# Lakonik/SSDNeRF

Measured on NVIDIA H100. Metric: rays/sec (128^2 render) & DDIM triplanes/sec, higher is better.
Workload: dtype fp16 tensor-core UNet (fp32 accumulate), fp32 renderer

## Files before the change

### include/ssdnerf_b200.h

```cpp
#ifndef SSDNERF_B200_H_
#define SSDNERF_B200_H_

#include <stdint.h>
#include <stddef.h>

#ifdef __cplusplus
extern "C" {
#endif

#define SSDNERF_API __attribute__((visibility("default")))

#define SSDNERF_OK 0
#define SSDNERF_ERR_CUDA (-1)
#define SSDNERF_ERR_ARG (-2)
#define SSDNERF_ERR_ARCH (-3)

SSDNERF_API const char* ssdnerf_last_error(void);
SSDNERF_API int ssdnerf_version(void);
SSDNERF_API int ssdnerf_compiled_arch(void);
SSDNERF_API unsigned long long ssdnerf_launch_count(void);

SSDNERF_API int ssdnerf_near_far_from_aabb(const float* rays_o, const float* rays_d, const float* aabb, uint32_t N, float min_near,
                               float* nears, float* fars, void* stream);
SSDNERF_API int ssdnerf_sph_from_ray(const float* rays_o, const float* rays_d, float radius, uint32_t N, float* coords, void* stream);
SSDNERF_API int ssdnerf_morton3D(const int* coords, uint32_t N, int* indices, void* stream);
SSDNERF_API int ssdnerf_morton3D_invert(const int* indices, uint32_t N, int* coords, void* stream);
SSDNERF_API int ssdnerf_packbits(const void* grid, int grid_is_half, uint32_t N, float thresh, uint8_t* bitfield, void* stream);
SSDNERF_API int ssdnerf_march_rays_train(const float* rays_o, const float* rays_d, const uint8_t* grid, float bound, float dt_gamma,
                             uint32_t max_steps, uint32_t N, uint32_t C, uint32_t H, uint32_t M, const float* nears,
                             const float* fars, float* xyzs, float* dirs, float* deltas, int* rays, int* counter,
                             const float* noises, void* stream);
SSDNERF_API int ssdnerf_composite_rays_train_forward(const float* sigmas, const float* rgbs, const float* deltas, const int* rays,
                                         uint32_t M, uint32_t N, float T_thresh, float* weights_sum, float* depth,
                                         float* image, void* stream);
SSDNERF_API int ssdnerf_composite_rays_train_backward(const float* grad_weights_sum, const float* grad_image, const float* sigmas,
                                          const float* rgbs, const float* deltas, const int* rays, const float* weights_sum,
                                          const float* image, uint32_t M, uint32_t N, float T_thresh, float* grad_sigmas,
                                          float* grad_rgbs, void* stream);
SSDNERF_API int ssdnerf_march_rays(uint32_t n_alive, uint32_t n_step, const int* rays_alive, const float* rays_t, const float* rays_o,
                       const float* rays_d, float bound, float dt_gamma, uint32_t max_steps, uint32_t C, uint32_t H,
                       const uint8_t* grid, const float* nears, const float* fars, float* xyzs, float* dirs, float* deltas,
                       const float* noises, void* stream);
SSDNERF_API int ssdnerf_composite_rays(uint32_t n_alive, uint32_t n_step, float T_thresh, int* rays_alive, float* rays_t,
                           const float* sigmas, const float* rgbs, const float* deltas, float* weights_sum, float* depth,
                           float* image, void* stream);
SSDNERF_API int ssdnerf_sh_encode_forward(const float* inputs, float* outputs, uint32_t B, uint32_t D, uint32_t C, int calc_grad_inputs,
                              float* dy_dx, void* stream);
SSDNERF_API int ssdnerf_sh_encode_backward(const float* grad, const float* inputs, uint32_t B, uint32_t D, uint32_t C, const float* dy_dx,
                               float* grad_inputs, void* stream);


#define SSDNERF_DEC_P 0
#define SSDNERF_DEC_S 1

SSDNERF_API size_t ssdnerf_decoder_blob_floats(int variant);

SSDNERF_API size_t ssdnerf_planes_bytes(int variant, uint32_t B, uint32_t Hp, uint32_t Wp);
SSDNERF_API int ssdnerf_pack_planes(int variant, const float* code, uint32_t B, uint32_t C, uint32_t Hp, uint32_t Wp, void* planes,
                        void* stream);

SSDNERF_API int ssdnerf_point_decode(int variant, const void* planes, uint32_t plane_h, uint32_t plane_w, const float* decoder_blob,
                                     const float* xyzs, const float* dirs, const long long* scene_offsets, uint32_t num_scenes,
                                     unsigned long long num_points, float* sigmas, float* rgbs, void* stream);

typedef struct ssdnerf_render_args {
    int variant;
    uint32_t num_scenes;
    uint32_t rays_per_scene;
    const float* rays_o;
    const float* rays_d;
    const float* poses;
    const float* intrinsics;
    uint32_t num_views, img_h, img_w;
    const void* planes;
    uint32_t plane_h, plane_w;
    const uint8_t* bitfield;
    uint32_t grid_size;
    const float* decoder_blob;
    const float* dt_gamma;
    float bound, min_near, T_thresh, bg_color;
    uint32_t max_steps;
    int emulate_schedule;
    float* weights_sum;
    float* depth;
    float* image;
    float* rgb_blend;
    int32_t* num_samples;
    int32_t* voxel_trace;
    uint32_t trace_cap;
    void* workspace;
    size_t workspace_bytes;
} ssdnerf_render_args;

SSDNERF_API size_t ssdnerf_render_workspace_bytes(uint32_t num_scenes, uint32_t rays_per_scene, uint32_t max_steps);
SSDNERF_API int ssdnerf_render_fwd(const ssdnerf_render_args* args, void* stream);

typedef struct ssdnerf_render_train_args {
    int variant;
    uint32_t num_scenes, rays_per_scene;
    const float* rays_o;
    const float* rays_d;
    const float* noises;
    const void* planes;
    uint32_t plane_h, plane_w;
    const uint8_t* bitfield;
    uint32_t grid_size;
    const float* decoder_blob;
    const float* dt_gamma;
    float bound, min_near, T_thresh;
    uint32_t max_steps;
    float* weights_sum;
    float* depth;
    float* image;
    int32_t* num_samples;
    const float* grad_ws;
    const float* grad_image;
    float* grad_planes;
    uint32_t* counter;
    float* grad_decoder_blob;
} ssdnerf_render_train_args;

SSDNERF_API int ssdnerf_cam_rays(const float* poses, const float* intrinsics, uint32_t B, uint32_t V, uint32_t h, uint32_t w,
                     float* rays_o, float* rays_d, void* stream);
SSDNERF_API int ssdnerf_render_train_fwd(const ssdnerf_render_train_args* args, void* stream);
SSDNERF_API int ssdnerf_render_train_bwd(const ssdnerf_render_train_args* args, void* stream);
SSDNERF_API int ssdnerf_unpack_plane_grads(const float* grad_planes, const float* code, float reg_coef, uint32_t B, uint32_t Hp, uint32_t Wp,
                               int accumulate, float* grad_code, void* stream);
SSDNERF_API int ssdnerf_mse_render_loss(const float* image, const float* weights_sum, const float* target, uint64_t rays, float bg_color,
                            float coef_loss, float coef_grad, float* out_rgb , float* grad_image, float* grad_ws,
                            float* loss , void* stream);

SSDNERF_API size_t ssdnerf_density_workspace_bytes(uint32_t num_scenes, uint32_t grid_size);
SSDNERF_API int ssdnerf_density_update(int variant, const void* planes, uint32_t plane_h, uint32_t plane_w, const float* decoder_blob,
                           uint32_t num_scenes, uint32_t grid_size, float bound,
                           const float* jitter,
                           float decay, void* density_grid, int grid_is_half, void* workspace, void* stream);
SSDNERF_API int ssdnerf_density_pack(const void* density_grid, int grid_is_half, uint32_t num_scenes, uint32_t grid_size,
                         float density_thresh, uint8_t* bitfield, float* thresh_out ,
                         void* workspace, void* stream);

typedef struct ssdnerf_gemm_args {
    const void* a1; uint64_t a1_strides[3]; uint32_t k1;
    const void* a2; uint64_t a2_strides[3]; uint32_t k2;
    uint32_t d1, d2, d3, b1, b2, b3;
    uint32_t taps;
    const void* b; uint64_t b_strides[3]; uint32_t n, n_rows_b, bx2, bx3; uint32_t b_batched;
    uint32_t bn;
    float alpha;
    const float* bias_n;
    const void* residual;
    void* out; uint32_t out_f32; long long so1, so2, so3;
    float* qstats; uint32_t stats_hw;
    uint32_t algo;
    const int8_t* tap_offsets;
    uint32_t a_stride;
    uint32_t relu;
} ssdnerf_gemm_args;
SSDNERF_API int ssdnerf_gemm_f16(const ssdnerf_gemm_args* args, void* stream);

SSDNERF_API int ssdnerf_nchw_to_nhwc_f16(const float* x, uint32_t B, uint32_t C, uint32_t H, uint32_t W, uint32_t Cpad, void* out, void* stream);
SSDNERF_API int ssdnerf_gn_stats(const void* x1, uint32_t C1, const void* x2, uint32_t C2, uint32_t B, uint32_t HW, uint32_t groups,
                                 float* stats, void* stream);
SSDNERF_API int ssdnerf_gn_apply_q(const void* x1, uint32_t C1, const void* x2, uint32_t C2, uint32_t B, uint32_t HW, uint32_t groups,
                                   const float* q1, const float* q2, const float* gamma, const float* beta, const float* scale_shift,
                                   long long ss_batch_stride, float eps, int do_silu, void* out, void* stream);
SSDNERF_API int ssdnerf_gn_apply(const void* x1, uint32_t C1, const void* x2, uint32_t C2, uint32_t B, uint32_t HW, uint32_t groups,
                                 const float* stats, const float* gamma, const float* beta, const float* scale_shift,
                                 long long ss_batch_stride, float eps, int do_silu, void* out, void* stream);
SSDNERF_API int ssdnerf_flash_attn(const void* qkv, uint32_t B, uint32_t T, uint32_t heads, uint32_t ch, float scale, void* out, void* stream);
SSDNERF_API int ssdnerf_softmax_rows(const float* S, uint32_t rows, uint32_t T, void* P, void* stream);
SSDNERF_API int ssdnerf_transpose_v(const void* qkv, uint32_t B, uint32_t T, uint32_t heads, uint32_t ch, void* vt, void* stream);
SSDNERF_API int ssdnerf_ddim_update(float* x_t, const float* v, uint32_t B, uint32_t C, uint32_t H, uint32_t W, uint32_t Cv,
                                    const float* coef, const int* step_ptr, int clip, float clip_lo, float clip_hi, float* x0_out,
                                    void* next_in, uint32_t Cpad, void* stream);
SSDNERF_API int ssdnerf_ddpm_update(float* x_t, const float* v, uint32_t B, uint32_t C, uint32_t H, uint32_t W, uint32_t Cv,
                                    const float* coef, const int* step_ptr, const unsigned long long* seed_ptr, int clip, float clip_lo,
                                    float clip_hi, void* next_in, uint32_t Cpad, void* stream);
SSDNERF_API int ssdnerf_step_counter(int* step_ptr, int value, int set, void* stream);
SSDNERF_API int ssdnerf_select_row(const float* table, uint32_t row_elems, const int* step_ptr, float* dst, uint32_t copies, void* stream);

typedef struct ssdnerf_gn_bwd_args {
    const void* x1; uint32_t C1;
    const void* x2; uint32_t C2;
    uint32_t B, HW, groups;
    const float* stats; const float* stats2; int quad_stats;
    const float* gamma; const float* beta;
    const float* scale_shift; long long ss_batch_stride;
    float eps; int do_silu;
    const void* dy;
    const void* add;
    float* group_sums;
    void* dx1; void* dx2;
    float* channel_sums;
} ssdnerf_gn_bwd_args;
SSDNERF_API int ssdnerf_gn_bwd(const ssdnerf_gn_bwd_args* args, void* stream);
SSDNERF_API int ssdnerf_softmax_bwd_rows(const void* P, const float* dP, uint32_t rows, uint32_t T, void* dS, void* stream);
SSDNERF_API int ssdnerf_transpose_f16(const void* src, void* dst, uint32_t rows, uint32_t cols, long long row_stride, long long stride1,
                                      uint32_t n1, long long stride2, uint32_t n2, void* stream);
SSDNERF_API int ssdnerf_col2im_s2(const void* dcol, uint32_t B, uint32_t H, uint32_t W, uint32_t C, const void* add, void* dx, void* stream);
SSDNERF_API int ssdnerf_sum2x2(const void* dup, uint32_t B, uint32_t H, uint32_t W, uint32_t C, void* dx, void* stream);
SSDNERF_API int ssdnerf_add_f16(void* dst, const void* src, unsigned long long n, void* stream);
SSDNERF_API int ssdnerf_grad_scale(const float* g, unsigned long long n, float target, float* scale, void* stream);
SSDNERF_API int ssdnerf_grad_nchw_to_nhwc_f16(const float* g, uint32_t B, uint32_t C, uint32_t H, uint32_t W, uint32_t Cpad, const float* scale,
                                              void* out, void* stream);
SSDNERF_API int ssdnerf_grad_nhwc_to_nchw_f32(const float* dx, uint32_t B, uint32_t C, uint32_t H, uint32_t W, uint32_t Cpad, float* scale,
                                              float* out, void* stream);


typedef struct ssdnerf_wgrad_args {
    const void* gy; uint32_t gy_stride, gy_c0;
    const void* x; uint32_t x_stride, x_c0;
    float* dw; uint32_t dw_stride, dw_c0;
    uint32_t batch, out_h, out_w, in_h, in_w;
    uint32_t cout, cin;
    uint32_t taps;
    uint32_t stride;
    int up;
    uint32_t ksplit;
} ssdnerf_wgrad_args;
SSDNERF_API int ssdnerf_conv_wgrad_f16(const ssdnerf_wgrad_args* args, void* stream);
SSDNERF_API int ssdnerf_dropout_f16(void* x, unsigned long long n, unsigned long long seed, float p_drop, void* stream);
SSDNERF_API int ssdnerf_colsum_f16(const void* src, uint64_t rows, uint32_t stride, uint32_t c0, uint32_t channels, float* out, void* stream);

SSDNERF_API int ssdnerf_ssim_f32(const float* pred, const float* target, uint32_t n, uint32_t h, uint32_t w, float* out, void* stream);
SSDNERF_API int ssdnerf_lpips_prep_f16(const float* pred, const float* target, uint32_t m, uint32_t h, uint32_t w, void* out, void* stream);
SSDNERF_API uint32_t ssdnerf_lpips_tap_partials(uint32_t m, uint32_t h, uint32_t w, uint32_t c, int pool);
SSDNERF_API int ssdnerf_lpips_tap_f16(const void* feat, uint32_t m, uint32_t h, uint32_t w, uint32_t c, const float* lin, float* partial,
                                     void* pooled, float* out, void* stream);

SSDNERF_API size_t ssdnerf_mc_workspace_bytes(uint32_t nx, uint32_t ny, uint32_t nz);
SSDNERF_API int ssdnerf_mc_count(const float* u, uint32_t nx, uint32_t ny, uint32_t nz, double threshold, void* workspace,
                                 unsigned long long* counts , void* stream);
SSDNERF_API int ssdnerf_mc_emit(const float* u, uint32_t nx, uint32_t ny, uint32_t nz, double threshold, const void* workspace,
                                double* vertices, long long* triangles, void* stream);
SSDNERF_API int ssdnerf_mc_case_table(uint8_t* tri_count_host, uint8_t* tri_host);

SSDNERF_API int ssdnerf_incep_prep_f16(const float* x, uint32_t n, uint32_t h, uint32_t w, void* out, uint8_t* u8, void* stream);
SSDNERF_API int ssdnerf_incep_conv_f16(const void* x, uint32_t n, uint32_t h, uint32_t w, uint32_t cin, uint32_t x_stride, const void* weight,
                                       const float* bias, uint32_t cout, uint32_t kh, uint32_t kw, uint32_t stride, uint32_t pad_h,
                                       uint32_t pad_w, int relu, void* y, uint32_t y_stride, void* stream);
#define SSDNERF_POOL_MAX_S2 0
#define SSDNERF_POOL_AVG_S1 1
#define SSDNERF_POOL_MAX_S1 2
SSDNERF_API int ssdnerf_incep_pool_f16(const void* x, uint32_t n, uint32_t h, uint32_t w, uint32_t c, uint32_t x_stride, int mode, void* y,
                                       uint32_t y_stride, void* stream);
SSDNERF_API int ssdnerf_incep_mean_f16(const void* x, uint32_t n, uint32_t hw, uint32_t c, float* out, void* stream);

#define SSDNERF_PNG_SEGMENT_BYTES 16384
SSDNERF_API size_t ssdnerf_png_workspace_bytes(uint32_t n, uint32_t h, uint32_t w);
SSDNERF_API size_t ssdnerf_png_output_bound(uint32_t n, uint32_t h, uint32_t w);
SSDNERF_API int ssdnerf_png_encode_views(const float* pred, const float* real, uint32_t n, uint32_t h, uint32_t w_view, void* workspace,
                                        size_t workspace_bytes, uint8_t* out, size_t out_bytes, unsigned long long* offsets,
                                        void* stream);
SSDNERF_API int ssdnerf_png_encode_maps(const float* maps, uint32_t n, uint32_t h, uint32_t w, float vmin, float vrange, void* workspace,
                                       size_t workspace_bytes, uint8_t* out, size_t out_bytes, unsigned long long* offsets,
                                       void* stream);
SSDNERF_API int ssdnerf_png_viridis(uint8_t* rgb_host);

#define SSDNERF_PNG_OK 0
#define SSDNERF_PNG_TRUNCATED 1
#define SSDNERF_PNG_BAD_ZLIB_HEADER 2
#define SSDNERF_PNG_BAD_BLOCK_TYPE 3
#define SSDNERF_PNG_BAD_STORED_LEN 4
#define SSDNERF_PNG_BAD_CODE_LENGTHS 5
#define SSDNERF_PNG_BAD_SYMBOL 6
#define SSDNERF_PNG_BAD_DISTANCE 7
#define SSDNERF_PNG_TOO_MUCH_DATA 8
#define SSDNERF_PNG_TOO_LITTLE_DATA 9
#define SSDNERF_PNG_BAD_FILTER 10
#define SSDNERF_PNG_BAD_ADLER 11
#define SSDNERF_PNG_BAD_DESC 12
typedef struct {
    uint64_t stream_offset;
    uint64_t palette_offset;
    uint64_t work_offset;
    uint64_t out_offset;
    uint32_t stream_bytes;
    uint32_t h, w;
    int32_t color_type;
} ssdnerf_png_desc;
SSDNERF_API size_t ssdnerf_png_decode_workspace_bytes(uint32_t h, uint32_t w, int color_type);
SSDNERF_API int ssdnerf_png_decode(const uint8_t* streams, size_t stream_bytes, const ssdnerf_png_desc* desc, uint32_t n, void* workspace,
                                   size_t workspace_bytes, float* out, size_t out_floats, int32_t* status, void* stream);
SSDNERF_API int ssdnerf_png_decode_host(const uint8_t* stream_host, size_t stream_bytes, uint32_t h, uint32_t w, int color_type,
                                        const uint8_t* palette_host, float* out_host, int32_t* status_host);

#ifdef __cplusplus
}
#endif
#endif
```

### ssdnerf_b200/_lib.py

```python
import ctypes
import os

import torch

_HERE = os.path.dirname(os.path.abspath(__file__))
_PATH = os.path.join(_HERE, 'libssdnerf_b200.so')
_lib = None

c_void_p = ctypes.c_void_p
c_u32 = ctypes.c_uint32
c_f32 = ctypes.c_float
c_double = ctypes.c_double
c_int = ctypes.c_int
c_size_t = ctypes.c_size_t
c_longlong = ctypes.c_longlong


class SSDNeRFNativeError(RuntimeError):
    pass


class RenderArgs(ctypes.Structure):
    _fields_ = [
        ('variant', c_int), ('num_scenes', c_u32), ('rays_per_scene', c_u32),
        ('rays_o', c_void_p), ('rays_d', c_void_p),
        ('poses', c_void_p), ('intrinsics', c_void_p),
        ('num_views', c_u32), ('img_h', c_u32), ('img_w', c_u32),
        ('planes', c_void_p), ('plane_h', c_u32), ('plane_w', c_u32),
        ('bitfield', c_void_p), ('grid_size', c_u32),
        ('decoder_blob', c_void_p), ('dt_gamma', c_void_p),
        ('bound', c_f32), ('min_near', c_f32), ('T_thresh', c_f32), ('bg_color', c_f32),
        ('max_steps', c_u32), ('emulate_schedule', c_int),
        ('weights_sum', c_void_p), ('depth', c_void_p), ('image', c_void_p), ('rgb_blend', c_void_p),
        ('num_samples', c_void_p), ('voxel_trace', c_void_p), ('trace_cap', c_u32),
        ('workspace', c_void_p), ('workspace_bytes', c_size_t),
    ]


class RenderTrainArgs(ctypes.Structure):
    _fields_ = [
        ('variant', c_int), ('num_scenes', c_u32), ('rays_per_scene', c_u32),
        ('rays_o', c_void_p), ('rays_d', c_void_p), ('noises', c_void_p),
        ('planes', c_void_p), ('plane_h', c_u32), ('plane_w', c_u32),
        ('bitfield', c_void_p), ('grid_size', c_u32),
        ('decoder_blob', c_void_p), ('dt_gamma', c_void_p),
        ('bound', c_f32), ('min_near', c_f32), ('T_thresh', c_f32),
        ('max_steps', c_u32),
        ('weights_sum', c_void_p), ('depth', c_void_p), ('image', c_void_p), ('num_samples', c_void_p),
        ('grad_ws', c_void_p), ('grad_image', c_void_p), ('grad_planes', c_void_p),
        ('counter', c_void_p), ('grad_decoder_blob', c_void_p),
    ]


def lib():
    global _lib
    if _lib is None:
        if not os.path.exists(_PATH):
            raise SSDNeRFNativeError(
                f'{_PATH} not found: build it with `python -m ssdnerf_b200.build` '
                '(there is no CPU / PyTorch fallback for the hot path)')
        L = ctypes.CDLL(_PATH)
        L.ssdnerf_last_error.restype = ctypes.c_char_p
        for name in ('ssdnerf_decoder_blob_floats', 'ssdnerf_planes_bytes', 'ssdnerf_render_workspace_bytes',
                     'ssdnerf_density_workspace_bytes', 'ssdnerf_unet_workspace_bytes'):
            if hasattr(L, name):
                getattr(L, name).restype = c_size_t
        L.ssdnerf_mc_workspace_bytes.argtypes = [c_u32, c_u32, c_u32]
        L.ssdnerf_mc_workspace_bytes.restype = c_size_t
        L.ssdnerf_mc_count.argtypes = [c_void_p, c_u32, c_u32, c_u32, c_double, c_void_p, c_void_p, c_void_p]
        L.ssdnerf_mc_emit.argtypes = [c_void_p, c_u32, c_u32, c_u32, c_double, c_void_p, c_void_p, c_void_p, c_void_p]
        L.ssdnerf_mc_case_table.argtypes = [c_void_p, c_void_p]
        for name in ('ssdnerf_png_workspace_bytes', 'ssdnerf_png_output_bound'):
            getattr(L, name).argtypes = [c_u32, c_u32, c_u32]
            getattr(L, name).restype = c_size_t
        L.ssdnerf_png_encode_views.argtypes = [c_void_p, c_void_p, c_u32, c_u32, c_u32, c_void_p, c_size_t, c_void_p, c_size_t,
                                               c_void_p, c_void_p]
        L.ssdnerf_png_encode_maps.argtypes = [c_void_p, c_u32, c_u32, c_u32, c_f32, c_f32, c_void_p, c_size_t, c_void_p, c_size_t,
                                              c_void_p, c_void_p]
        L.ssdnerf_png_viridis.argtypes = [c_void_p]
        L.ssdnerf_png_decode_workspace_bytes.argtypes = [c_u32, c_u32, c_int]
        L.ssdnerf_png_decode_workspace_bytes.restype = c_size_t
        L.ssdnerf_png_decode.argtypes = [c_void_p, c_size_t, c_void_p, c_u32, c_void_p, c_size_t, c_void_p, c_size_t, c_void_p, c_void_p]
        L.ssdnerf_png_decode_host.argtypes = [ctypes.c_char_p, c_size_t, c_u32, c_u32, c_int, ctypes.c_char_p, c_void_p, c_void_p]
        _lib = L
    return _lib


def check(code):
    if code != 0:
        raise SSDNeRFNativeError(f'libssdnerf_b200 error {code}: {lib().ssdnerf_last_error().decode()}')


def ptr(t):
    if t is None:
        return None
    assert t.is_contiguous(), 'native ops need contiguous tensors'
    return c_void_p(t.data_ptr())


def stream_ptr(device=None):
    return c_void_p(torch.cuda.current_stream(device).cuda_stream)


def require_cuda(*tensors):
    cur = None
    for t in tensors:
        if t is None:
            continue
        if not t.is_cuda:
            raise SSDNeRFNativeError('ssdnerf_b200 ops run on CUDA tensors only (no CPU fallback)')
        if cur is None:
            cur = torch.cuda.current_device()
        if t.device.index != cur:
            raise SSDNeRFNativeError(f'tensor on cuda:{t.device.index} but the current device is cuda:{cur}: the library launches on the '
                                     'current device (one GPU per process, or wrap the call in torch.cuda.device(...))')
```

### ssdnerf_b200/csrc/gemm_tc.cu

```cuda
#include "common.cuh"
#include "tc_common.cuh"
#include "conv_row_epilogue.cuh"
#include "../../include/ssdnerf_b200.h"
#include <cuda_fp16.h>
#include <cstdio>

namespace ssdnerf {
using namespace tc;

constexpr int kGemmThreads = 384;
constexpr int kMaxBiasN = 2048;
constexpr int kBM = 128, kBK = 64;
constexpr int kABytes = kBM * kBK * 2;

struct GemmParams {
    uint32_t b1, b2, b3;
    uint32_t d1, d2, d3;
    uint32_t T1, T2, T3;
    uint32_t tiles_n;
    uint32_t taps;
    int8_t tap_ox[9], tap_oy[9];
    uint32_t a_stride;
    uint32_t kc1, kc2;
    uint32_t n_valid;
    uint32_t b_batched;
    uint32_t vec2;
    float alpha;
    const float* bias_n;
    const __half* residual;
    void* out;
    uint32_t out_f32;
    long long so1, so2, so3;
    float* qstats;
    uint32_t stats_hw;
    uint32_t k1, k2;
};

template <int BN>
struct GemmCfg {
    static constexpr int kBBytes = BN * kBK * 2;
    static constexpr int kStageBytes = kABytes + kBBytes;
    static constexpr int kStages = (192 * 1024 / kStageBytes) > 8 ? 8 : (192 * 1024 / kStageBytes);
    static constexpr size_t kSmem = (size_t)kStages * kStageBytes + 1024  + 256  + 1024  +
                                    kMaxBiasN * 4 ;
};

template <int BN, bool KT, bool RELU = false>
__global__ void __launch_bounds__(kGemmThreads, 1)
k_gemm_tc(const __grid_constant__ CUtensorMap mapA1, const __grid_constant__ CUtensorMap mapA2,
          const __grid_constant__ CUtensorMap mapB, const GemmParams p) {
    using Cfg = GemmCfg<BN>;
    extern __shared__ uint8_t smem_raw[];
    uint8_t* smem = reinterpret_cast<uint8_t*>(((uintptr_t)smem_raw + 1023) & ~(uintptr_t)1023);
    uint8_t* sA = smem;
    uint8_t* sB = smem + Cfg::kStages * kABytes;
    uint64_t* full = reinterpret_cast<uint64_t*>(smem + Cfg::kStages * Cfg::kStageBytes);
    uint64_t* empty = full + Cfg::kStages;
    float* qacc = reinterpret_cast<float*>(smem + Cfg::kStages * Cfg::kStageBytes + 256);
    float* sbias = qacc + 256;

    const int warp = threadIdx.x >> 5, lane = threadIdx.x & 31, wg = warp >> 2;
    const uint32_t tiles_m = p.T1 * p.T2 * p.T3;
    const uint32_t total_tiles = tiles_m * p.tiles_n;
    const uint32_t iters = p.taps * (p.kc1 + p.kc2);
    const uint32_t tile0 = blockIdx.x;
    const uint32_t tile_step = gridDim.x;

    if (threadIdx.x == 0) {
        prefetch_tmap(&mapA1); prefetch_tmap(&mapA2); prefetch_tmap(&mapB);
        for (int i = 0; i < Cfg::kStages; ++i) { mbar_init(&full[i], 1); mbar_init(&empty[i], 8); }
        fence_mbar_init();
    }
    for (int i = threadIdx.x; i < BN; i += kGemmThreads) qacc[i] = 0.0f;
    if (p.bias_n) for (uint32_t i = threadIdx.x; i < p.n_valid; i += kGemmThreads) sbias[i] = __ldg(p.bias_n + i);
    __syncthreads();
    pdl_trigger();
    pdl_wait();

    if (wg == 0) {
        setmaxnreg_dec<40>();
        if (threadIdx.x == 0) {
            uint32_t stage = 0, phase = 0;
            for (uint32_t tile = tile0; tile < total_tiles; tile += tile_step) {
                const uint32_t m_tile = tile % tiles_m, n_tile = tile / tiles_m;
                const uint32_t t1 = m_tile % p.T1, t2 = (m_tile / p.T1) % p.T2, t3 = m_tile / (p.T1 * p.T2);
                for (uint32_t tap = 0; tap < p.taps; ++tap) {
                    const int ox = p.tap_ox[tap], oy = p.tap_oy[tap];
                    for (uint32_t j = 0; j < p.kc1 + p.kc2; ++j) {
                        mbar_wait(&empty[stage], phase ^ 1);
                        const bool first = j < p.kc1;
                        const int ak = (int)((first ? j : j - p.kc1) * kBK), a1 = (int)(t1 * p.b1 * p.a_stride) + ox, a2 = (int)(t2 * p.b2 * p.a_stride) + oy, a3 = (int)(t3 * p.b3);
                        mbar_expect_tx(&full[stage], (uint32_t)Cfg::kStageBytes);
                        tma_load_4d(sA + stage * kABytes, first ? &mapA1 : &mapA2, &full[stage], ak, a1, a2, a3);
                        const int bk = KT ? (first ? ak : (int)p.k1 + ak) : (int)(j * kBK);
                        tma_load_4d(sB + stage * Cfg::kBBytes, &mapB, &full[stage], bk, (int)(n_tile * BN),
                                    p.b_batched ? (int)t2 : (int)tap, p.b_batched ? (int)t3 : 0);
                        if (++stage == Cfg::kStages) { stage = 0; phase ^= 1; }
                    }
                }
            }
        }
    } else {
        setmaxnreg_inc<232>();
        const uint32_t cw = (uint32_t)wg - 1u;
        const uint32_t wq = (uint32_t)warp & 3u;
        const uint32_t rbase = cw * 64u + wq * 16u + ((uint32_t)lane >> 2);
        const uint32_t cq = (uint32_t)lane & 3u;
        uint32_t stage = 0, phase = 0;
        float acc[BN / 2];
        auto release = [&](uint32_t s) { if (lane == 0) mbar_arrive(&empty[s]); };
        for (uint32_t tile = tile0; tile < total_tiles; tile += tile_step) {
            const uint32_t m_tile = tile % tiles_m, n_tile = tile / tiles_m;
            const uint32_t t1 = m_tile % p.T1, t2 = (m_tile / p.T1) % p.T2, t3 = m_tile / (p.T1 * p.T2);
#pragma unroll
            for (int i = 0; i < BN / 2; ++i) acc[i] = 0.0f;
            uint32_t prev = 0;
            uint32_t jc = 0;
            for (uint32_t it = 0; it < iters; ++it) {
                mbar_wait(&full[stage], phase);
                const uint64_t a_desc = make_desc_sw128(smem_u32(sA + stage * kABytes + cw * 64 * 128));
                const uint64_t b_desc = make_desc_sw128(smem_u32(sB + stage * Cfg::kBBytes));
                wgmma_fence();
                fence_regs(acc);
                uint32_t nk = kBK / 16;
                if constexpr (KT) {
                    const uint32_t kx = jc < p.kc1 ? p.k1 - jc * kBK : p.k2 - (jc - p.kc1) * kBK;
                    nk = kx >= (uint32_t)kBK ? kBK / 16 : (kx + 15u) / 16u;
                    if (++jc == p.kc1 + p.kc2) jc = 0;
                }
#pragma unroll
                for (uint32_t k = 0; k < kBK / 16; ++k) {
                    if (KT && k >= nk) break;
                    if constexpr (BN == 256) wgmma_ss_n256(acc, a_desc + 2 * k, b_desc + 2 * k, 1u);
                    else if constexpr (BN == 128) wgmma_ss_n128(acc, a_desc + 2 * k, b_desc + 2 * k, 1u);
                    else if constexpr (BN == 160) wgmma_ss_n160(acc, a_desc + 2 * k, b_desc + 2 * k, 1u);
                    else if constexpr (BN == 80) wgmma_ss_n80(acc, a_desc + 2 * k, b_desc + 2 * k, 1u);
                    else if constexpr (BN == 48) wgmma_ss_n48(acc, a_desc + 2 * k, b_desc + 2 * k, 1u);
                    else if constexpr (BN == 40) wgmma_ss_n40(acc, a_desc + 2 * k, b_desc + 2 * k, 1u);
                    else if constexpr (BN == 16) wgmma_ss_n16(acc, a_desc + 2 * k, b_desc + 2 * k, 1u);
                    else wgmma_ss_n64(acc, a_desc + 2 * k, b_desc + 2 * k, 1u);
                }
                wgmma_commit();
                fence_regs(acc);
                wgmma_wait<1>();
                if (it > 0) release(prev);
                prev = stage;
                if (++stage == Cfg::kStages) { stage = 0; phase ^= 1; }
            }
            wgmma_wait<0>();
            fence_regs(acc);
            if (iters > 0) release(prev);

            long long off[2]; bool rok[2];
#pragma unroll
            for (int h = 0; h < 2; ++h) {
                const uint32_t row = rbase + 8u * h;
                const uint32_t i1 = row % p.b1, i2 = (row / p.b1) % p.b2, i3 = row / (p.b1 * p.b2);
                const uint32_t g1 = t1 * p.b1 + i1, g2 = t2 * p.b2 + i2, g3 = t3 * p.b3 + i3;
                rok[h] = m_tile < tiles_m && g1 < p.d1 && g2 < p.d2 && g3 < p.d3;
                off[h] = (long long)g1 * p.so1 + (long long)g2 * p.so2 + (long long)g3 * p.so3 + (long long)n_tile * BN;
            }
            uint32_t slot = 0, img0 = 0;
            if (p.qstats) {
                const uint32_t r0 = cw * 64u;
                const uint32_t j1 = r0 % p.b1, j3 = r0 / (p.b1 * p.b2);
                img0 = p.stats_hw ? (t1 * p.b1) / p.stats_hw : t3 * p.b3;
                slot = ((p.stats_hw ? (t1 * p.b1 + j1) / p.stats_hw : t3 * p.b3 + j3) - img0) & 1u;
            }
#pragma unroll
            for (int i = 0; i < BN / 8; ++i) {
                const uint32_t c0 = 8u * i + 2u * cq;
                const uint32_t ncol = n_tile * BN + c0;
                const bool okc0 = ncol < p.n_valid, okc1 = ncol + 1 < p.n_valid;
                float su = 0.0f, sq = 0.0f;
#pragma unroll
                for (int h = 0; h < 2; ++h) {
                    float v0 = acc[4 * i + 2 * h] * p.alpha, v1 = acc[4 * i + 2 * h + 1] * p.alpha;
                    if (!rok[h] || !okc0) continue;
                    if (p.bias_n) { v0 += sbias[ncol]; if (okc1) v1 += sbias[ncol + 1]; }
                    const long long o = off[h] + c0;
                    if (p.residual) {
                        if (p.vec2 && okc1) {
                            const float2 r = __half22float2(*reinterpret_cast<const __half2*>(p.residual + o));
                            v0 += r.x; v1 += r.y;
                        } else {
                            v0 += __half2float(p.residual[o]);
                            if (okc1) v1 += __half2float(p.residual[o + 1]);
                        }
                    }
                    if constexpr (RELU) { v0 = fmaxf(v0, 0.0f); v1 = fmaxf(v1, 0.0f); }
                    if (p.out_f32) {
                        float* op = reinterpret_cast<float*>(p.out) + o;
                        if (p.vec2 && okc1) *reinterpret_cast<float2*>(op) = make_float2(v0, v1);
                        else { op[0] = v0; if (okc1) op[1] = v1; }
                    } else {
                        __half* op = reinterpret_cast<__half*>(p.out) + o;
                        if (p.vec2 && okc1) *reinterpret_cast<__half2*>(op) = __floats2half2_rn(v0, v1);
                        else { op[0] = __float2half_rn(v0); if (okc1) op[1] = __float2half_rn(v1); }
                    }
                    if (!okc1) v1 = 0.0f;
                    su += v0 + v1; sq = fmaf(v0, v0, fmaf(v1, v1, sq));
                }
                if (p.qstats) {
                    frag_quad_reduce(su, sq);
                    if ((lane & ~2) == 0) {
                        float* qa = qacc + (slot * (BN / 4) + 2 * i + (lane >> 1)) * 2;
                        atomicAdd(qa, su); atomicAdd(qa + 1, sq);
                    }
                }
            }
            if (p.qstats) {
                asm volatile("bar.sync 1, 256;" ::: "memory");
                const uint32_t et = threadIdx.x - 128;
                const uint32_t nq = p.n_valid / 4;
                for (uint32_t i = et; i < (uint32_t)BN; i += 256) {
                    const float val = qacc[i];
                    const uint32_t sl = i / (BN / 2), qd = (i % (BN / 2)) >> 1, st = i & 1u;
                    const uint32_t gq = n_tile * (BN / 4) + qd;
                    if (val != 0.0f && gq < nq) atomicAdd(p.qstats + ((size_t)(img0 + sl) * nq + gq) * 2 + st, val);
                    qacc[i] = 0.0f;
                }
                asm volatile("bar.sync 1, 256;" ::: "memory");
            }
        }
    }
    __syncthreads();
}

typedef CUresult (*PFN_encodeTiled)(CUtensorMap*, CUtensorMapDataType, cuuint32_t, void*, const cuuint64_t*, const cuuint64_t*,
                                    const cuuint32_t*, const cuuint32_t*, CUtensorMapInterleave, CUtensorMapSwizzle,
                                    CUtensorMapL2promotion, CUtensorMapFloatOOBfill);

static PFN_encodeTiled get_encode() {
    static PFN_encodeTiled fn = nullptr;
    if (!fn) {
        void* p = nullptr;
        cudaDriverEntryPointQueryResult qres;
        if (cudaGetDriverEntryPoint("cuTensorMapEncodeTiled", &p, cudaEnableDefault, &qres) != cudaSuccess || !p) return nullptr;
        fn = (PFN_encodeTiled)p;
    }
    return fn;
}

static int make_map_4d(CUtensorMap* m, const void* base, uint64_t K, uint64_t e1, uint64_t e2, uint64_t e3, uint64_t s1, uint64_t s2,
                       uint64_t s3, uint32_t x1, uint32_t x2, uint32_t x3, uint32_t trav = 1) {
    PFN_encodeTiled enc = get_encode();
    if (!enc) return set_error_msg(SSDNERF_ERR_CUDA, "cuTensorMapEncodeTiled entry point not found");
    if (((uintptr_t)base & 15u) || (s1 & 15u) || (s2 & 15u) || (s3 & 15u))
        return set_error_msg(SSDNERF_ERR_ARG, "gemm: TMA operands need 16-byte aligned base and strides");
    cuuint64_t dims[4] = {K, e1, e2, e3};
    cuuint64_t strides[3] = {s1, s2, s3};
    cuuint32_t box[4] = {64, x1 * trav, x2 * trav, x3};
    cuuint32_t estr[4] = {1, trav, trav, 1};
    const CUresult r = enc(m, CU_TENSOR_MAP_DATA_TYPE_FLOAT16, 4, const_cast<void*>(base), dims, strides, box, estr,
                           CU_TENSOR_MAP_INTERLEAVE_NONE, CU_TENSOR_MAP_SWIZZLE_128B, CU_TENSOR_MAP_L2_PROMOTION_L2_256B,
                           CU_TENSOR_MAP_FLOAT_OOB_FILL_NONE);
    if (r != CUDA_SUCCESS) {
        char buf[200];
        snprintf(buf, sizeof(buf), "cuTensorMapEncodeTiled failed (%d): dims {%llu,%llu,%llu,%llu} box {64,%u,%u,%u}", (int)r,
                 (unsigned long long)K, (unsigned long long)e1, (unsigned long long)e2, (unsigned long long)e3, x1, x2, x3);
        return set_error_msg(SSDNERF_ERR_CUDA, buf);
    }
    return 0;
}

int make_map_4d_box(CUtensorMap* m, const void* base, uint64_t K, uint64_t e1, uint64_t e2, uint64_t e3, uint64_t s1, uint64_t s2, uint64_t s3,
                    uint32_t x1, uint32_t x2, uint32_t x3) {
    return make_map_4d(m, base, K, e1, e2, e3, s1, s2, s3, x1, x2, x3);
}
int conv_row2_launch(const ssdnerf_gemm_args* a, int sms, cudaStream_t stream);

template <int BN, bool KT = false, bool RELU = false>
static int launch_gemm(const CUtensorMap& mA1, const CUtensorMap& mA2, const CUtensorMap& mB, const GemmParams& p, int sms,
                       cudaStream_t stream) {
    using Cfg = GemmCfg<BN>;
    static DeviceOnce attr;
    if (attr.first()) {
        SSDNERF_CUDA_OK(cudaFuncSetAttribute(k_gemm_tc<BN, KT, RELU>, cudaFuncAttributeMaxDynamicSharedMemorySize, (int)Cfg::kSmem));
    }
    const uint32_t total = p.T1 * p.T2 * p.T3 * p.tiles_n;
    cudaLaunchConfig_t cfg{};
    cfg.gridDim = dim3(total < (uint32_t)sms ? total : (uint32_t)sms);
    cfg.blockDim = dim3(kGemmThreads);
    cfg.dynamicSmemBytes = Cfg::kSmem;
    cfg.stream = stream;
    cudaLaunchAttribute at[1];
    at[0].id = cudaLaunchAttributeProgrammaticStreamSerialization;
    at[0].val.programmaticStreamSerializationAllowed = pdl_enabled() ? 1 : 0;
    cfg.attrs = at; cfg.numAttrs = 1;
    SSDNERF_CUDA_OK(cudaLaunchKernelEx(&cfg, k_gemm_tc<BN, KT, RELU>, mA1, mA2, mB, p));
    SSDNERF_LAUNCH_OK();
    return 0;
}

}

using namespace ssdnerf;

extern "C" int ssdnerf_gemm_f16(const ssdnerf_gemm_args* a, void* stream_) {
    cudaStream_t stream = (cudaStream_t)stream_;
    if (!a || !a->a1 || !a->b || !a->out) return set_error_msg(SSDNERF_ERR_ARG, "gemm: a1, b and out are required");
    const bool kt = a->algo == 3;
    if (kt) {
        if (a->k1 == 0 || a->k1 % 8 || (a->a2 && (a->k2 == 0 || a->k2 % 8)))
            return set_error_msg(SSDNERF_ERR_ARG, "gemm (narrow): K extents must be multiples of 8");
    } else if (a->k1 == 0 || a->k1 % 64 || a->k2 % 64) {
        return set_error_msg(SSDNERF_ERR_ARG, "gemm: K extents must be multiples of 64");
    }
    if (a->b1 * a->b2 * a->b3 != 128) return set_error_msg(SSDNERF_ERR_ARG, "gemm: b1*b2*b3 must be 128");
    if (a->taps < 1 || a->taps > 9) return set_error_msg(SSDNERF_ERR_ARG, "gemm: taps must be in [1, 9]");
    if (a->taps != 1 && a->taps != 9 && !a->tap_offsets) return set_error_msg(SSDNERF_ERR_ARG, "gemm: taps other than 1 / 9 need tap_offsets");
    if (a->taps > 1 && a->b_batched) return set_error_msg(SSDNERF_ERR_ARG, "gemm: conv taps and batched B are exclusive");
    if (a->a_stride > 2) return set_error_msg(SSDNERF_ERR_ARG, "gemm: a_stride must be 0 / 1 / 2");
    const uint32_t a_stride = a->a_stride == 2 ? 2u : 1u;
    if (a_stride == 2 && (a->b1 * 2 > 256 || a->b2 * 2 > 256)) return set_error_msg(SSDNERF_ERR_ARG, "gemm: stride-2 boxes exceed the 256-element TMA limit");
    if (a->n == 0 || a->d1 == 0 || a->d2 == 0 || a->d3 == 0) return 0;
    int dev = 0, sms = 0;
    SSDNERF_CUDA_OK(cudaGetDevice(&dev));
    SSDNERF_CUDA_OK(cudaDeviceGetAttribute(&sms, cudaDevAttrMultiProcessorCount, dev));
    if (a->algo != 1 && !kt && !a->relu && a->taps == 9 && !a->tap_offsets && a_stride == 1 && a->d1 == 128 && a->b1 == 128 && a->b2 == 1 && a->b3 == 1 && a->n == 128 && !a->out_f32 && !a->b_batched &&
        (a->d2 % 2) == 0 && a->alpha == 1.0f && (a->bn == 0 || a->bn == 128) && a->so1 == 128 && a->so2 == 128 * 128 &&
        a->so3 == (long long)a->d2 * 128 * 128 && (!a->qstats || a->stats_hw == 0) && (a->n_rows_b == 0 || a->n_rows_b >= 128))
        return ssdnerf::conv_row2_launch(a, sms, stream);
    if (a->algo == 2) return set_error_msg(SSDNERF_ERR_ARG, "gemm: algo 2 (row-pair convolution) needs taps 9, 128-pixel rows, 128 output channels, fp16 output");
    int bn = (int)a->bn;
    if (kt) {
        const int cand[6] = {256, 160, 80, 48, 40, 16};
        if (a->relu) {
            if (bn && bn != 16) return set_error_msg(SSDNERF_ERR_ARG, "gemm (narrow): relu needs bn 0 or 16");
            bn = 16;
        } else if (bn) {
            bool ok = false;
            for (int c : cand) ok |= c == bn;
            if (!ok) return set_error_msg(SSDNERF_ERR_ARG, "gemm (narrow): bn must be 16, 40, 48, 80, 160 or 256");
        } else {
            for (int c : cand) if (a->n % (uint32_t)c == 0) { bn = c; break; }
            if (!bn) {
                uint32_t best = 0xFFFFFFFFu;
                for (int c : cand) { const uint32_t w = div_up(a->n, (uint32_t)c) * (uint32_t)c; if (w < best) { best = w; bn = c; } }
            }
        }
    } else if (!bn) {
        const uint32_t tiles_m = div_up(a->d1, a->b1) * div_up(a->d2, a->b2) * div_up(a->d3, a->b3);
        double best = 1e30;
        const int cand[3] = {256, 128, 64};
        const double eff[3] = {1.0, 0.80, 0.50};
        for (int i = 0; i < 3; ++i) {
            if (cand[i] > 64 && (uint32_t)cand[i] / 2 >= a->n) continue;
            const uint32_t tiles = tiles_m * div_up(a->n, (uint32_t)cand[i]);
            const double t = (double)div_up(tiles, (uint32_t)sms) * cand[i] / eff[i];
            if (t < best) { best = t; bn = cand[i]; }
        }
    }
    if (!kt && bn != 64 && bn != 128 && bn != 256) return set_error_msg(SSDNERF_ERR_ARG, "gemm: bn must be 64, 128 or 256");

    GemmParams p{};
    p.b1 = a->b1; p.b2 = a->b2; p.b3 = a->b3; p.d1 = a->d1; p.d2 = a->d2; p.d3 = a->d3;
    p.T1 = div_up(a->d1, a->b1); p.T2 = div_up(a->d2, a->b2); p.T3 = div_up(a->d3, a->b3);
    p.tiles_n = div_up(a->n, (uint32_t)bn);
    p.a_stride = a_stride;
    for (uint32_t t = 0; t < 9; ++t) {
        if (a->tap_offsets) { p.tap_ox[t] = a->tap_offsets[2 * t]; p.tap_oy[t] = a->tap_offsets[2 * t + 1]; }
        else if (a->taps == 9) { p.tap_ox[t] = (int8_t)((int)(t % 3) - 1); p.tap_oy[t] = (int8_t)((int)(t / 3) - 1); }
        else { p.tap_ox[t] = 0; p.tap_oy[t] = 0; }
    }
    p.taps = a->taps; p.kc1 = div_up(a->k1, 64u); p.kc2 = a->a2 ? div_up(a->k2, 64u) : 0;
    p.k1 = a->k1; p.k2 = a->a2 ? a->k2 : 0; p.n_valid = a->n; p.b_batched = a->b_batched;
    p.alpha = a->alpha; p.bias_n = a->bias_n; p.residual = (const __half*)a->residual; p.out = a->out; p.out_f32 = a->out_f32;
    p.so1 = a->so1; p.so2 = a->so2; p.so3 = a->so3;
    p.qstats = a->qstats; p.stats_hw = a->stats_hw;
    const uintptr_t pair_align = a->out_f32 ? 8u : 4u;
    p.vec2 = ((a->so1 | a->so2 | a->so3) & 1) == 0 && ((uintptr_t)a->out % pair_align) == 0 && ((uintptr_t)a->residual & 3u) == 0;
    if (a->bias_n && a->n > (uint32_t)kMaxBiasN) return set_error_msg(SSDNERF_ERR_ARG, "gemm: bias vectors longer than 2048 are not supported");
    if (a->qstats && (a->n % 4)) return set_error_msg(SSDNERF_ERR_ARG, "gemm: quad statistics need n % 4 == 0");
    if (a->qstats && !a->stats_hw && a->b3 > 2) return set_error_msg(SSDNERF_ERR_ARG, "gemm: fused quad statistics cover at most 2 images per 128-row tile (b3 <= 2)");
    if (a->qstats && a->stats_hw && (a->stats_hw % 64)) return set_error_msg(SSDNERF_ERR_ARG, "gemm: stats_hw must be a multiple of 64");
    const uint64_t ktot = (uint64_t)a->k1 + (a->a2 ? a->k2 : 0);

    CUtensorMap mA1, mA2, mB;
    const uint64_t e1 = (uint64_t)a->d1 * a_stride, e2 = (uint64_t)a->d2 * a_stride;
    if (int e = make_map_4d(&mA1, a->a1, a->k1, e1, e2, a->d3, a->a1_strides[0], a->a1_strides[1], a->a1_strides[2], a->b1, a->b2, a->b3, a_stride)) return e;
    if (a->a2) {
        if (int e = make_map_4d(&mA2, a->a2, a->k2, e1, e2, a->d3, a->a2_strides[0], a->a2_strides[1], a->a2_strides[2], a->b1, a->b2, a->b3, a_stride)) return e;
    } else {
        mA2 = mA1;
    }
    if (int e = make_map_4d(&mB, a->b, ktot, a->n_rows_b ? a->n_rows_b : a->n, a->bx2 ? a->bx2 : 1, a->bx3 ? a->bx3 : 1, a->b_strides[0],
                            a->b_strides[1], a->b_strides[2], (uint32_t)bn, 1, 1)) return e;

    if (a->relu) {
        if (kt) return launch_gemm<16, true, true>(mA1, mA2, mB, p, sms, stream);
        if (bn == 256) return launch_gemm<256, false, true>(mA1, mA2, mB, p, sms, stream);
        if (bn == 128) return launch_gemm<128, false, true>(mA1, mA2, mB, p, sms, stream);
        return launch_gemm<64, false, true>(mA1, mA2, mB, p, sms, stream);
    }
    if (kt) {
        switch (bn) {
            case 256: return launch_gemm<256, true>(mA1, mA2, mB, p, sms, stream);
            case 160: return launch_gemm<160, true>(mA1, mA2, mB, p, sms, stream);
            case 80: return launch_gemm<80, true>(mA1, mA2, mB, p, sms, stream);
            case 48: return launch_gemm<48, true>(mA1, mA2, mB, p, sms, stream);
            case 40: return launch_gemm<40, true>(mA1, mA2, mB, p, sms, stream);
            default: return launch_gemm<16, true>(mA1, mA2, mB, p, sms, stream);
        }
    }
    if (bn == 256) return launch_gemm<256>(mA1, mA2, mB, p, sms, stream);
    if (bn == 128) return launch_gemm<128>(mA1, mA2, mB, p, sms, stream);
    return launch_gemm<64>(mA1, mA2, mB, p, sms, stream);
}
```

### ssdnerf_b200/unet.py

```python
import math
from copy import deepcopy

import torch
import torch.nn as nn

from . import _lib as N
from . import unet_ops as U
from .registry import MODULES


_GN_GROUPS = [32]


def _gn(c):
    return nn.GroupNorm(_GN_GROUPS[0], c, eps=1e-5)


class _ResBlockParams(nn.Module):

    def __init__(self, cin, cout, emb_ch, dropout=0.0):
        super().__init__()
        self.conv_1 = nn.Sequential(_gn(cin), nn.SiLU(), nn.Conv2d(cin, cout, 3, padding=1))
        self.norm_with_embedding = nn.Module()
        self.norm_with_embedding.norm = _gn(cout)
        self.norm_with_embedding.embedding_layer = nn.Sequential(nn.SiLU(), nn.Linear(emb_ch, 2 * cout))
        conv_2 = [nn.SiLU(), nn.Dropout(dropout), nn.Conv2d(cout, cout, 3, padding=1)] if dropout > 0 \
            else [nn.SiLU(), nn.Conv2d(cout, cout, 3, padding=1)]
        self.conv_2 = nn.Sequential(*conv_2)
        if cin != cout:
            self.shortcut = nn.Conv2d(cin, cout, 1)
        self.cin, self.cout = cin, cout
        nn.init.zeros_(self.conv_2[-1].weight)
        nn.init.zeros_(self.conv_2[-1].bias)


class _AttnParams(nn.Module):

    def __init__(self, c, num_heads):
        super().__init__()
        self.norm = _gn(c)
        self.qkv = nn.Conv1d(c, 3 * c, 1)
        self.proj = nn.Conv1d(c, c, 1)
        self.c, self.num_heads = c, num_heads
        nn.init.zeros_(self.proj.weight)
        nn.init.zeros_(self.proj.bias)


class _DownParams(nn.Module):
    def __init__(self, c):
        super().__init__()
        self.downsample = nn.Conv2d(c, c, 3, 2, 1)
        self.c = c


class _UpParams(nn.Module):
    def __init__(self, c):
        super().__init__()
        self.conv = nn.Conv2d(c, c, 3, 1, 1)
        self.c = c


class _TimeEmbedding(nn.Module):

    def __init__(self, base, emb_ch):
        super().__init__()
        self.blocks = nn.Sequential(nn.Linear(base, emb_ch), nn.SiLU(), nn.Linear(emb_ch, emb_ch))
        self.base = base

    def forward(self, t):
        half = self.base // 2
        freqs = torch.exp(-math.log(10000) * torch.arange(half, dtype=torch.float32, device=t.device) / half)
        args = t[:, None].float() * freqs[None]
        return self.blocks(torch.cat([torch.cos(args), torch.sin(args)], dim=-1))


@MODULES.register_module()
class DenoisingUnetMod(nn.Module):

    def __init__(self, image_size, in_channels=3, concat_cond_channels=0, base_channels=128, resblocks_per_downsample=3,
                 num_timesteps=1000, use_rescale_timesteps=True, dropout=0, embedding_channels=-1, num_classes=0,
                 channels_cfg=None, groups=1, norm_cfg=dict(type='GN', num_groups=32), act_cfg=dict(type='SiLU', inplace=False),
                 shortcut_kernel_size=1, use_scale_shift_norm=False, num_heads=4, time_embedding_mode='sin',
                 time_embedding_cfg=None, resblock_cfg=dict(type='DenoisingResBlockMod'),
                 attention_cfg=dict(type='MultiHeadAttentionMod'), downsample_conv=True, upsample_conv=True,
                 downsample_cfg=dict(type='DenoisingDownsampleMod'), upsample_cfg=dict(type='DenoisingUpsampleMod'),
                 attention_res=[16, 8], pretrained=None):
        super().__init__()
        unsupported = []
        if groups != 1: unsupported.append('groups != 1')
        if num_classes != 0: unsupported.append('class conditioning')
        if not use_scale_shift_norm: unsupported.append('use_scale_shift_norm=False')
        if shortcut_kernel_size != 1: unsupported.append('shortcut_kernel_size != 1')
        if not (downsample_conv and upsample_conv): unsupported.append('pool / bare-interpolate resampling')
        if norm_cfg.get('type') != 'GN': unsupported.append('norm other than GroupNorm')
        if act_cfg.get('type') != 'SiLU': unsupported.append('activation other than SiLU')
        if time_embedding_mode != 'sin': unsupported.append('time_embedding_mode != sin')
        if unsupported:
            raise NotImplementedError('ssdnerf_b200.DenoisingUnetMod covers the configurations the reference ships; unsupported: '
                                      + ', '.join(unsupported))
        if not isinstance(channels_cfg, (list, tuple)):
            raise ValueError(f'Only support list for `channels_cfg`, receive {type(channels_cfg)}')
        self.num_classes, self.num_timesteps, self.use_rescale_timesteps = num_classes, num_timesteps, use_rescale_timesteps
        self.num_groups = int(norm_cfg.get('num_groups', 32))
        _GN_GROUPS[0] = self.num_groups
        self.out_channels = in_channels
        self.in_channels = in_channels
        self.concat_cond_channels = concat_cond_channels
        if isinstance(image_size, int):
            image_size = [image_size, image_size]
        assert len(image_size) == 2, 'The length of `image_size` should be 2.'
        self.image_size = list(image_size)
        self.channel_factor_list = list(channels_cfg)
        self.num_heads = num_heads
        self.base_channels = base_channels
        self.dropout = float(dropout)
        emb_ch = base_channels * 4 if embedding_channels == -1 else embedding_channels
        self.embedding_channels = emb_ch
        self.time_embedding = _TimeEmbedding(base_channels, emb_ch)

        attention_scale = [min(image_size) // int(res) for res in attention_res]
        scale = 1
        self.in_blocks = nn.ModuleList([nn.Sequential(nn.Conv2d(in_channels + concat_cond_channels, base_channels, 3, 1, padding=1))])
        self.in_channels_list = [base_channels]
        cin = base_channels
        for level, factor in enumerate(self.channel_factor_list):
            cin = base_channels if level == 0 else base_channels * self.channel_factor_list[level - 1]
            cout = base_channels * factor
            for _ in range(resblocks_per_downsample):
                layers = [_ResBlockParams(cin, cout, emb_ch, dropout)]
                cin = cout
                if scale in attention_scale:
                    layers.append(_AttnParams(cin, num_heads))
                self.in_channels_list.append(cin)
                self.in_blocks.append(nn.Sequential(*layers))
            if level != len(self.channel_factor_list) - 1:
                self.in_blocks.append(nn.Sequential(_DownParams(cin)))
                self.in_channels_list.append(cin)
                scale *= 2
        self.mid_blocks = nn.Sequential(_ResBlockParams(cin, cin, emb_ch, dropout), _AttnParams(cin, num_heads),
                                        _ResBlockParams(cin, cin, emb_ch, dropout))
        in_list = deepcopy(self.in_channels_list)
        self.out_blocks = nn.ModuleList()
        for level, factor in enumerate(self.channel_factor_list[::-1]):
            for idx in range(resblocks_per_downsample + 1):
                layers = [_ResBlockParams(cin + in_list.pop(), base_channels * factor, emb_ch, dropout)]
                cin = base_channels * factor
                if scale in attention_scale:
                    layers.append(_AttnParams(cin, num_heads))
                if level != len(self.channel_factor_list) - 1 and idx == resblocks_per_downsample:
                    layers.append(_UpParams(cin))
                    scale //= 2
                self.out_blocks.append(nn.Sequential(*layers))
        self.out = nn.Module()
        self.out.conv = nn.Conv2d(cin, in_channels, 3, padding=1)
        self.out.gn = _gn(cin)
        _GN_GROUPS[0] = 32
        self._engine = None
        self._engine_key = None

    def engine(self, batch, device=None, hw=None):
        device = device or next(self.parameters()).device
        hw = tuple(int(v) for v in (hw if hw is not None else self.image_size))
        key = (batch, str(device), hw, tuple(p._version for p in self.parameters()))
        if self._engine is None or self._engine_key != key:
            old = self._engine
            self._engine = UNetEngine(self, batch, device, hw)
            if old is not None and self._engine_key is not None and self._engine_key[:3] == key[:3]:
                self._engine.bufs = old.bufs
            self._engine_key = key
        return self._engine

    def refresh_weights(self):
        self._engine = None
        self._engine_key = None

    def embedding(self, t):
        if self.use_rescale_timesteps:
            t = t.float() * (1000.0 / self.num_timesteps)
        return self.time_embedding(t)

    def forward(self, x_t, t, label=None, concat_cond=None, return_noise=False):
        if label is not None:
            raise NotImplementedError('class-conditional embedding is not built (num_classes == 0 in every reference config)')
        N.require_cuda(x_t)
        h = x_t
        if self.concat_cond_channels > 0:
            h = torch.cat([h, concat_cond], dim=1)
        B = h.shape[0]
        if t.dim() == 0 or t.numel() != B:
            t = t.expand(B)
        if torch.is_grad_enabled() and any(p.requires_grad for p in self.parameters()):
            from .unet_train import forward_with_weight_grads
            return forward_with_weight_grads(self, h, t)
        if torch.is_grad_enabled() and h.requires_grad:
            if self.concat_cond_channels > 0:
                raise NotImplementedError('input gradients with concat_cond are not built (unused by the shipped configs)')
            return _UNetInputGrad.apply(h, self, t)
        with torch.no_grad():
            eng = self.engine(B, h.device, h.shape[-2:])
            eng.set_embedding(self.embedding(t.to(h.device)))
            v = eng.forward_nchw(h.float().contiguous())
            return v.permute(0, 3, 1, 2)[:, :self.out_channels].contiguous()


class _UNetInputGrad(torch.autograd.Function):

    @staticmethod
    def forward(ctx, x_t, module, t):
        B = x_t.shape[0]
        eng = module.engine(B, x_t.device, x_t.shape[-2:])
        eng.set_embedding(module.embedding(t.to(x_t.device)))
        eng.load_input_nchw(x_t.detach().float().contiguous())
        v = eng.forward_nhwc(save=True)
        ctx.eng, ctx.token, ctx.C = eng, eng.fwd_token, module.out_channels
        return v.permute(0, 3, 1, 2)[:, :module.out_channels].contiguous()

    @staticmethod
    def backward(ctx, grad_v):
        eng = ctx.eng
        if eng.fwd_token != ctx.token:
            raise RuntimeError('UNet input gradient: the engine ran another forward before this backward (activations overwritten)')
        return eng.backward_nchw(grad_v.contiguous().float()), None, None


def unet_widths(m):
    return sorted({m.base_channels * f for f in m.channel_factor_list} | {m.base_channels})


def is_narrow(m):
    return any(w % 64 for w in unet_widths(m))


class UNetEngine:

    CPAD_IN = 64

    def __init__(self, m: DenoisingUnetMod, batch, device, hw=None):
        self.m, self.B, self.dev = m, batch, torch.device(device)
        widths = unet_widths(m)
        self.groups = m.num_groups
        if any(w % 16 for w in widths) or any(w % self.groups for w in widths):
            raise NotImplementedError(f'native UNet engine: channel widths must be multiples of 16 and of the GroupNorm group count; got '
                                      f'widths {widths}, {self.groups} groups')
        self.narrow = is_narrow(m)
        attn_widths = sorted({p.c for p in m.modules() if isinstance(p, _AttnParams)})
        if any(c % m.num_heads or (c // m.num_heads) % 8 for c in attn_widths):
            raise NotImplementedError(f'native UNet engine: attention head widths must be multiples of 8; got widths {attn_widths} over '
                                      f'{m.num_heads} heads')
        self.H, self.W = (int(v) for v in (hw if hw is not None else m.image_size))
        self.bufs = {}
        self.cin_total = m.in_channels + m.concat_cond_channels
        if self.narrow:
            self.CPAD_IN = max(16, (self.cin_total + 15) // 16 * 16)
        assert self.cin_total <= self.CPAD_IN
        nw = self.narrow
        dev = self.dev
        f32 = lambda p: p.detach().float().contiguous().to(dev)
        self.ops = []
        self.res_blocks = []
        self.n_norm = 0

        def res(p):
            d = dict(cin=p.cin, cout=p.cout, g1=f32(p.conv_1[0].weight), b1=f32(p.conv_1[0].bias),
                     w1=U.pack_conv_weight(p.conv_1[2].weight, narrow=nw).to(dev), c1b=f32(p.conv_1[2].bias),
                     g2=f32(p.norm_with_embedding.norm.weight), b2=f32(p.norm_with_embedding.norm.bias),
                     w2=U.pack_conv_weight(p.conv_2[-1].weight, narrow=nw).to(dev), c2b=f32(p.conv_2[-1].bias),
                     emb_w=f32(p.norm_with_embedding.embedding_layer[1].weight), emb_b=f32(p.norm_with_embedding.embedding_layer[1].bias),
                     n1=self._norm_slot(), n2=self._norm_slot(), idx=len(self.res_blocks), mod=p)
            if hasattr(p, 'shortcut'):
                d['ws'] = U.pack_linear_weight(p.shortcut.weight, narrow=nw).to(dev)
                d['wsb'] = f32(p.shortcut.bias)
            self.res_blocks.append(d)
            return ('res', d)

        def attn(p):
            return ('attn', dict(c=p.c, heads=p.num_heads, g=f32(p.norm.weight), b=f32(p.norm.bias),
                                 wqkv=U.pack_linear_weight(p.qkv.weight, narrow=nw).to(dev), bqkv=f32(p.qkv.bias),
                                 wproj=U.pack_linear_weight(p.proj.weight, narrow=nw).to(dev), bproj=f32(p.proj.bias), n=self._norm_slot(),
                                 mod=p))

        def layer(p):
            if isinstance(p, _ResBlockParams): return res(p)
            if isinstance(p, _AttnParams): return attn(p)
            if isinstance(p, _DownParams):
                return ('down', dict(c=p.c, w=U.pack_conv_weight(p.downsample.weight, narrow=nw).to(dev), b=f32(p.downsample.bias), mod=p))
            if isinstance(p, _UpParams):
                return ('up', dict(c=p.c, w=U.pack_upconv_weight(p.conv.weight, narrow=nw).to(dev), b=f32(p.conv.bias), mod=p))
            raise TypeError(type(p))

        conv_in = m.in_blocks[0][0]
        self.conv_in = dict(w=U.pack_conv_weight(conv_in.weight, cin_pad=self.CPAD_IN).to(dev), b=f32(conv_in.bias), cout=conv_in.out_channels)
        self.in_seq = [[layer(p) for p in blk] for blk in list(m.in_blocks)[1:]]
        self.mid_seq = [layer(p) for p in m.mid_blocks]
        self.out_seq = [[layer(p) for p in blk] for blk in m.out_blocks]
        self.out_norm = dict(g=f32(m.out.gn.weight), b=f32(m.out.gn.bias), n=self._norm_slot(), c=m.out.gn.num_channels)
        self.out_conv = dict(w=U.pack_conv_weight(m.out.conv.weight, narrow=nw).to(dev), b=f32(m.out.conv.bias), cout=m.out.conv.out_channels)
        self.qarena = torch.zeros(4 * 1024 * 1024, dtype=torch.float32, device=dev)
        self.qoff = 0
        self.qslots = {}
        self._legacy_idx = 0
        self.ss_offsets, off = [], 0
        for d in self.res_blocks:
            self.ss_offsets.append(off)
            off += 2 * d['cout']
        self.ss_total = off
        self.ss_cur = torch.zeros(batch, self.ss_total, dtype=torch.float32, device=dev)
        self.saving, self.tape, self.fwd_token, self._bwd_packed = False, [], 0, False
        self.drop_p, self._drop_seed = float(m.dropout), None
        self.x_in = torch.zeros(batch, self.H, self.W, self.CPAD_IN, dtype=torch.float16, device=dev)
        self.v_out = torch.zeros(batch, self.H, self.W, self.out_conv['cout'], dtype=torch.float32, device=dev)

    def _norm_slot(self):
        self.n_norm += 1
        return self.n_norm - 1

    def _buf(self, key, shape, dtype=torch.float16):
        t = self.bufs.get(key)
        if t is None or tuple(t.shape) != tuple(shape) or t.dtype != dtype:
            t = torch.empty(*shape, dtype=dtype, device=self.dev)
            self.bufs[key] = t
        return t

    def scale_shift_rows(self, emb, live=False):
        e = torch.nn.functional.silu(emb.float())
        if live:
            lins = [d['mod'].norm_with_embedding.embedding_layer[1] for d in self.res_blocks]
            return torch.cat([torch.nn.functional.linear(e, l.weight.float(), l.bias.float()) for l in lins], dim=1)
        return torch.cat([torch.nn.functional.linear(e, d['emb_w'], d['emb_b']) for d in self.res_blocks], dim=1)

    def new_dropout_seed(self, training):
        self._drop_seed = int(torch.randint(0, 2 ** 62, (1,)).item()) if (training and self.drop_p > 0) else None

    def _dropout(self, a2, block_idx):
        if self._drop_seed is not None:
            U.dropout_f16(a2, self._drop_seed + 0x9E3779B97F4A7C15 * (block_idx + 1), self.drop_p)

    def set_embedding(self, emb):
        self.ss_cur.copy_(self.scale_shift_rows(emb))

    def _q(self, key, channels):
        if (channels // self.groups) % 4:
            return None
        t = self.qslots.get(key)
        if t is None:
            n = self.B * (channels // 4) * 2
            t = self.qarena[self.qoff:self.qoff + n].view(self.B, channels // 4, 2)
            self.qoff += (n + 63) // 64 * 64
            assert self.qoff <= self.qarena.numel()
            self.qslots[key] = t
        return t

    def _gn(self, x1, q1, x2, q2, gamma, beta, out, silu, ss_off=None):
        B, H, W, C1 = x1.shape
        C2 = x2.shape[-1] if x2 is not None else 0
        G = self.groups
        L, s = N.lib(), N.stream_ptr()
        ss = None
        if ss_off is not None:
            ss = N.c_void_p(self.ss_cur.data_ptr() + 4 * ss_off)
        if ((C1 + C2) // G) % 4 != 0 or q1 is None or (x2 is not None and q2 is None):
            self._legacy_idx += 1
            st = self._q(('legacy', self._legacy_idx), G * 4)
            N.check(L.ssdnerf_gn_stats(N.ptr(x1), N.c_u32(C1), N.ptr(x2), N.c_u32(C2), N.c_u32(B), N.c_u32(H * W), N.c_u32(G), N.ptr(st), s))
            N.check(L.ssdnerf_gn_apply(N.ptr(x1), N.c_u32(C1), N.ptr(x2), N.c_u32(C2), N.c_u32(B), N.c_u32(H * W), N.c_u32(G), N.ptr(st),
                                       N.ptr(gamma), N.ptr(beta), ss, N.c_longlong(self.ss_total), N.c_f32(1e-5), N.c_int(int(silu)),
                                       N.ptr(out), s))
            self._last_stats = (False, st, None)
            return out
        self._last_stats = (True, q1, q2)
        N.check(L.ssdnerf_gn_apply_q(N.ptr(x1), N.c_u32(C1), N.ptr(x2), N.c_u32(C2), N.c_u32(B), N.c_u32(H * W), N.c_u32(G), N.ptr(q1),
                                     N.ptr(q2), N.ptr(gamma), N.ptr(beta), ss, N.c_longlong(self.ss_total), N.c_f32(1e-5),
                                     N.c_int(int(silu)), N.ptr(out), s))
        return out

    def _res(self, d, x, skip, tag):
        (x, qx), (sk, qs) = x, (skip if skip is not None else (None, None))
        B, H, W, _ = x.shape
        cin, cout = d['cin'], d['cout']
        nw = self.narrow
        if 'ws' in d:
            sc = U.conv3x3_f16(x, d['ws'].unsqueeze(0), cout, bias=d['wsb'], x2=sk, taps=1, out=self._buf(('sc', H, cout), (B, H, W, cout)),
                               narrow=nw)
        else:
            if sk is not None:
                raise NotImplementedError('ResBlock with a skip concat but no shortcut convolution (cin + skip == cout) is not built')
            sc = x
        qh1 = self._q(('h1', tag), cout)
        qo = self._q(('res_out', tag), cout)
        a = self._gn(x, qx, sk, qs, d['g1'], d['b1'], self._buf(('a', H, cin), (B, H, W, cin)), True)
        st1 = self._last_stats
        h1 = U.conv3x3_f16(a, d['w1'], cout, bias=d['c1b'], out=self._buf(('h1', tag) if self.saving else ('h1', H, cout), (B, H, W, cout)),
                           qstats=qh1, narrow=nw)
        a2 = self._gn(h1, qh1, None, None, d['g2'], d['b2'], self._buf(('a2', H, cout), (B, H, W, cout)), True, self.ss_offsets[d['idx']])
        st2 = self._last_stats
        if self.saving:
            self._dropout(a2, d['idx'])
        out = U.conv3x3_f16(a2, d['w2'], cout, bias=d['c2b'], residual=sc, out=self._buf(('res_out', tag), (B, H, W, cout)), qstats=qo,
                            narrow=nw)
        if self.saving:
            self.tape.append(dict(kind='res', d=d, x=x, sk=sk, st1=st1, h1=h1, st2=st2, out=out, tag=tag))
        return out, qo

    def _attn(self, d, x, tag):
        x, qx = x
        B, H, W, c = x.shape
        T, heads = H * W, d['heads']
        ch = c // heads
        L, s = N.lib(), N.stream_ptr()
        xn = self._gn(x, qx, None, None, d['g'], d['b'], self._buf(('xn', T, c), (B, H, W, c)), False)
        st = self._last_stats
        qkv = U.linear_f16(xn.view(B * T, c), d['wqkv'], bias=d['bqkv'], n=3 * c,
                           out=self._buf(('qkv', tag) if self.saving else ('qkv', T, c), (B * T, 3 * c)), narrow=self.narrow)
        o = self._attn_core(qkv, B, T, c, heads, ('o', T, c))
        qo = self._q(('attn_out', tag), c) if T % 64 == 0 else None
        out = U.linear_f16(o.view(B * T, c), d['wproj'], bias=d['bproj'], residual=x.view(B * T, c), n=c,
                           out=self._buf(('attn_out', tag), (B * T, c)), qstats=qo, stats_hw=T, narrow=self.narrow).view(B, H, W, c)
        if self.saving:
            self.tape.append(dict(kind='attn', d=d, x=x, st=st, qkv=qkv.view(B, T, 3 * c), out=out, tag=tag))
        return out, qo

    def _attn_core(self, qkv, B, T, c, heads, out_key):
        ch = c // heads
        L, s = N.lib(), N.stream_ptr()
        if ch in (64, 128) and T % 64 == 0:
            return U.flash_attn(qkv.view(B, T, 3 * c), heads, 1.0 / math.sqrt(ch), out=self._buf(out_key, (B, T, c)))
        S = U.attn_scores(qkv.view(B, T, 3 * c), heads, scale=1.0 / math.sqrt(ch), out=self._buf(('S', T), (B, heads, T, T), torch.float32),
                          narrow=self.narrow)
        P = self._buf(('P', T), (B, heads, T, T))
        N.check(L.ssdnerf_softmax_rows(N.ptr(S), N.c_u32(B * heads * T), N.c_u32(T), N.ptr(P), s))
        vt = self._buf(('vt', T, c), (B, heads, ch, T))
        N.check(L.ssdnerf_transpose_v(N.ptr(qkv), N.c_u32(B), N.c_u32(T), N.c_u32(heads), N.c_u32(ch), N.ptr(vt), s))
        return U.attn_pv(P, vt, out=self._buf(out_key, (B, T, c)), narrow=self.narrow)

    def _down(self, d, x, tag):
        x, _ = x
        B, H, W, c = x.shape
        qo = self._q(('down_out', tag), c)
        out = U.conv3x3_s2_f16(x, d['w'], c, bias=d['b'], out=self._buf(('down_out', tag), (B, H // 2, W // 2, c)), qstats=qo, narrow=self.narrow)
        if self.saving:
            self.tape.append(dict(kind='down', d=d, x=x, out=out, tag=tag))
        return out, qo

    def _up(self, d, x, tag):
        x, _ = x
        B, H, W, c = x.shape
        qo = self._q(('up_out', tag), c)
        out = U.upconv3x3_f16(x, d['w'], c, bias=d['b'], out=self._buf(('up_out', tag), (B, 2 * H, 2 * W, c)), qstats=qo, narrow=self.narrow)
        if self.saving:
            self.tape.append(dict(kind='up', d=d, x=x, out=out, tag=tag))
        return out, qo

    def _run(self, layers, h, skip, tag):
        for li, (kind, d) in enumerate(layers):
            t = (tag, li)
            if kind == 'res':
                h = self._res(d, h, skip, t)
                skip = None
            elif kind == 'attn':
                h = self._attn(d, h, t)
            elif kind == 'down':
                h = self._down(d, h, t)
            elif kind == 'up':
                h = self._up(d, h, t)
        return h

    def forward_nhwc(self, save=False):
        self.saving, self.tape = bool(save), []
        self.fwd_token += 1
        self.qarena[:max(self.qoff, 1)].zero_()
        self._legacy_idx = 0
        q0 = self._q(('conv_in',), self.conv_in['cout'])
        h = (U.conv3x3_f16(self.x_in, self.conv_in['w'], self.conv_in['cout'], bias=self.conv_in['b'],
                           out=self._buf(('conv_in',), (self.B, self.H, self.W, self.conv_in['cout'])), qstats=q0, narrow=self.narrow), q0)
        if self.saving:
            self.tape.append(dict(kind='conv_in', out=h[0]))
        hs = [h]
        for i, layers in enumerate(self.in_seq):
            h = self._run(layers, h, None, ('in', i))
            hs.append(h)
        h = self._run(self.mid_seq, h, None, ('mid',))
        for j, layers in enumerate(self.out_seq):
            h = self._run(layers, h, hs.pop(), ('out', j))
        h, qh = h
        B, H, W, c = h.shape
        a = self._gn(h, qh, None, None, self.out_norm['g'], self.out_norm['b'], self._buf(('a', H, c), (B, H, W, c)), True)
        if self.saving:
            self.tape.append(dict(kind='out', x=h, st=self._last_stats))
        U.conv3x3_f16(a, self.out_conv['w'], self.out_conv['cout'], bias=self.out_conv['b'], out=self.v_out, narrow=self.narrow)
        self.saving = False
        return self.v_out

    def _pack_backward_weights(self):
        m, dev, nw = self.m, self.dev, self.narrow

        def params(seq, mods):
            for (kind, d), p in zip(seq, mods):
                if kind == 'res':
                    d['w1T'] = U.pack_conv_weight_dgrad(p.conv_1[2].weight, narrow=nw).to(dev)
                    d['w2T'] = U.pack_conv_weight_dgrad(p.conv_2[-1].weight, narrow=nw).to(dev)
                    if hasattr(p, 'shortcut'):
                        d['wsT'] = U.pack_linear_weight_dgrad(p.shortcut.weight, narrow=nw).to(dev)
                elif kind == 'attn':
                    d['wqkvT'] = U.pack_linear_weight_dgrad(p.qkv.weight, narrow=nw).to(dev)
                    d['wprojT'] = U.pack_linear_weight_dgrad(p.proj.weight, narrow=nw).to(dev)
                elif kind == 'down':
                    w = p.downsample.weight.detach().permute(0, 2, 3, 1).reshape(p.c, 9 * p.c)
                    d['wT'] = U.pack_linear_weight_dgrad(w, narrow=nw).to(dev)
                elif kind == 'up':
                    d['wT'] = U.pack_conv_weight_dgrad(p.conv.weight, narrow=nw).to(dev)

        for seq, blk in zip(self.in_seq, list(m.in_blocks)[1:]):
            params(seq, blk)
        params(self.mid_seq, m.mid_blocks)
        for seq, blk in zip(self.out_seq, m.out_blocks):
            params(seq, blk)
        self.conv_in['wT'] = U.pack_conv_weight_dgrad(m.in_blocks[0][0].weight, narrow=nw).to(dev)
        self.out_conv['wT'] = U.pack_conv_weight_dgrad(m.out.conv.weight, cout_pad=self.CPAD_IN).to(dev)
        self._bwd_packed = True

    GRAD_TARGET = 1024.0
    GRAD_RETRIES = 4

    def backward_nchw(self, grad_v, weight_grads=False):
        from .unet_train import WeightGradPass
        B, C, H, W = grad_v.shape
        L, s = N.lib(), N.stream_ptr()
        scale = self._buf(('bwd', 'scale'), (4,), torch.float32)
        g_in = self._buf(('bwd', 'g_in'), (B, H, W, self.CPAD_IN))
        out = torch.empty(B, self.cin_total, H, W, dtype=torch.float32, device=self.dev)

        def walk(target, check=False):
            N.check(L.ssdnerf_grad_scale(N.ptr(grad_v), N.ctypes.c_ulonglong(grad_v.numel()), N.c_f32(target), N.ptr(scale), s))
            N.check(L.ssdnerf_grad_nchw_to_nhwc_f16(N.ptr(grad_v), N.c_u32(B), N.c_u32(C), N.c_u32(H), N.c_u32(W), N.c_u32(self.CPAD_IN),
                                                    N.ptr(scale), N.ptr(g_in), s))
            wg = WeightGradPass(self) if weight_grads else None
            dx = self.backward_nhwc(g_in, wg=wg, check=check)
            N.check(L.ssdnerf_grad_nhwc_to_nchw_f32(N.ptr(dx), N.c_u32(B), N.c_u32(self.cin_total), N.c_u32(H), N.c_u32(W),
                                                    N.c_u32(self.CPAD_IN), N.ptr(scale), N.ptr(out), s))
            return wg

        for k in range(self.GRAD_RETRIES + 1):
            target = self.GRAD_TARGET / 8 ** k
            wg = walk(target)
            grad_v_bad, dx_bad = scale[2:].tolist()
            if grad_v_bad or not dx_bad:
                break
        else:
            walk(target, check=True)
            raise N.SSDNeRFNativeError(f'UNet backward: d x_t is not finite at loss-scale target {target} although d loss / d v is')
        if wg is not None:
            grads, d_ss = wg.finish(scale[1])
            return out, grads, d_ss
        return out

    def _layer_name(self, r):
        if r['kind'] == 'out':
            return 'out'
        if r['kind'] == 'conv_in':
            return 'in_blocks.0.0'
        return next(n for n, mod in self.m.named_modules() if mod is r['d']['mod'])

    def backward_nhwc(self, g_v, wg=None, check=False):
        if not self.tape or self.tape[-1]['kind'] != 'out':
            raise N.SSDNeRFNativeError('UNet backward needs a preceding forward_nhwc(save=True)')
        if not self._bwd_packed:
            self._pack_backward_weights()
        L, s = N.lib(), N.stream_ptr
        nw, G = self.narrow, self.groups
        grads = {}

        def gb(name, idx, shape, dtype=torch.float16):
            return self._buf(('bwd', name, idx), shape, dtype)

        def acc(t, g):
            k = t.data_ptr()
            old = grads.get(k)
            if old is not None:
                N.check(L.ssdnerf_add_f16(N.ptr(g), N.ptr(old), N.ctypes.c_ulonglong(g.numel()), s()))
            grads[k] = g

        gsum = self._buf(('bwd', 'gsum'), (self.B * 64,), torch.float32)
        dx_in = None
        for idx in range(len(self.tape) - 1, -1, -1):
            r = self.tape[idx]
            kind = r['kind']
            if kind == 'out':
                x = r['x']
                B, H, W, c = x.shape
                d_a = U.conv3x3_f16(g_v, self.out_conv['wT'], c, out=gb('d_a', (H, c), (B, H, W, c)), narrow=nw)
                dh = gb('dx', idx, (B, H, W, c))
                cs = wg.csum(c) if wg else None
                U.gn_bwd(x, None, r['st'], self.out_norm['g'], self.out_norm['b'], d_a, dh, silu=True, gsum=gsum, csum=cs, groups=G)
                if wg:
                    wg.out(r, g_v, cs)
                acc(x, dh)
            elif kind == 'res':
                d, x, sk, h1, out = r['d'], r['x'], r['sk'], r['h1'], r['out']
                g = grads.pop(out.data_ptr())
                B, H, W, C1 = x.shape
                C2 = sk.shape[-1] if sk is not None else 0
                cin, cout = d['cin'], d['cout']
                d_a2 = U.conv3x3_f16(g, d['w2T'], cout, out=gb('d_a2', (H, cout), (B, H, W, cout)), narrow=nw)
                self._dropout(d_a2, d['idx'])
                d_h1 = gb('d_h1', (H, cout), (B, H, W, cout))
                ss = N.c_void_p(self.ss_cur.data_ptr() + 4 * self.ss_offsets[d['idx']])
                cs2 = wg.csum(cout) if wg else None
                U.gn_bwd(h1, None, r['st2'], d['g2'], d['b2'], d_a2, d_h1, scale_shift_ptr=ss, ss_batch_stride=self.ss_total, silu=True, gsum=gsum,
                         csum=cs2, groups=G)
                if wg:
                    wg.res_second(r, g, cs2)
                d_a = U.conv3x3_f16(d_h1, d['w1T'], cin, out=gb('d_a', (H, cin), (B, H, W, cin)), narrow=nw)
                if 'wsT' in d:
                    add = U.conv3x3_f16(g, d['wsT'].unsqueeze(0), cin, taps=1, out=gb('d_sc', (H, cin), (B, H, W, cin)), narrow=nw)
                else:
                    assert sk is None and cin == cout
                    add = g
                dx = gb('dx', idx, (B, H, W, C1))
                dsk = gb('dsk', idx, (B, H, W, C2)) if sk is not None else None
                cs1 = wg.csum(cin) if wg else None
                U.gn_bwd(x, sk, r['st1'], d['g1'], d['b1'], d_a, dx, dsk, add=add, silu=True, gsum=gsum, csum=cs1, groups=G)
                if wg:
                    wg.res_first(r, g, d_h1, cs1)
                acc(x, dx)
                if sk is not None:
                    acc(sk, dsk)
            elif kind == 'attn':
                d, x, qkv, out = r['d'], r['x'], r['qkv'], r['out']
                g = grads.pop(out.data_ptr())
                B, H, W, c = x.shape
                T, heads = H * W, d['heads']
                d_o = U.linear_f16(g.view(B * T, c), d['wprojT'], n=c, out=gb('d_o', (T, c), (B * T, c)), narrow=nw)
                dqkv = U.attn_backward(qkv, d_o.view(B, T, c), heads, 1.0 / math.sqrt(c // heads),
                                       lambda name, shape, dtype: gb('att_' + name, (T, c), shape, dtype), narrow=nw)
                d_xn = U.linear_f16(dqkv.view(B * T, 3 * c), d['wqkvT'], n=c, out=gb('d_xn', (T, c), (B * T, c)), narrow=nw)
                dx = gb('dx', idx, (B, H, W, c))
                cs = wg.csum(c) if wg else None
                U.gn_bwd(x, None, r['st'], d['g'], d['b'], d_xn.view(B, H, W, c), dx, add=g, silu=False, gsum=gsum, csum=cs, groups=G)
                if wg:
                    wg.attn(r, g, dqkv, cs)
                acc(x, dx)
            elif kind == 'down':
                d, x, out = r['d'], r['x'], r['out']
                g = grads.pop(out.data_ptr())
                B, H, W, c = x.shape
                if wg:
                    wg.down(r, g)
                M = B * (H // 2) * (W // 2)
                dcol = U.linear_f16(g.view(M, c), d['wT'], n=9 * c, out=gb('dcol', (H, c), (M, 9 * c)), narrow=nw)
                dx = gb('dx', idx, (B, H, W, c))
                old = grads.pop(x.data_ptr(), None)
                N.check(L.ssdnerf_col2im_s2(N.ptr(dcol), N.c_u32(B), N.c_u32(H), N.c_u32(W), N.c_u32(c), N.ptr(old), N.ptr(dx), s()))
                grads[x.data_ptr()] = dx
            elif kind == 'up':
                d, x, out = r['d'], r['x'], r['out']
                g = grads.pop(out.data_ptr())
                B, H, W, c = x.shape
                if wg:
                    wg.up(r, g)
                dup = U.conv3x3_f16(g, d['wT'], c, out=gb('dup', (H, c), (B, 2 * H, 2 * W, c)), narrow=nw)
                dx = gb('dx', idx, (B, H, W, c))
                N.check(L.ssdnerf_sum2x2(N.ptr(dup), N.c_u32(B), N.c_u32(H), N.c_u32(W), N.c_u32(c), N.ptr(dx), s()))
                acc(x, dx)
            elif kind == 'conv_in':
                g = grads.pop(r['out'].data_ptr())
                if wg:
                    wg.conv_in(r, g)
                dx_in = self._buf(('bwd', 'dx_in'), (self.B, self.H, self.W, self.CPAD_IN), torch.float32)
                U.conv3x3_f16(g, self.conv_in['wT'], self.cin_total, out=dx_in, narrow=nw)
            if check and not all(bool(torch.isfinite(t).all()) for t in list(grads.values()) + ([dx_in] if dx_in is not None else [])):
                raise N.SSDNeRFNativeError(f'UNet backward: the fp16 gradients overflow at layer `{self._layer_name(r)}` even with the '
                                           f'loss scale lowered {8 ** self.GRAD_RETRIES}x (forward activations or weights out of range?)')
        assert not grads, 'dangling gradients in the UNet tape'
        return dx_in

    def load_input_nchw(self, x):
        B, C, H, W = x.shape
        N.check(N.lib().ssdnerf_nchw_to_nhwc_f16(N.ptr(x), N.c_u32(B), N.c_u32(C), N.c_u32(H), N.c_u32(W), N.c_u32(self.CPAD_IN),
                                                 N.ptr(self.x_in), N.stream_ptr()))

    def forward_nchw(self, x):
        self.load_input_nchw(x)
        return self.forward_nhwc()
```

### ssdnerf_b200/unet_ops.py

```python
import ctypes

import torch

from . import _lib as N

c_u64 = ctypes.c_uint64
c_ll = ctypes.c_longlong


class GemmArgs(ctypes.Structure):
    _fields_ = [
        ('a1', N.c_void_p), ('a1_strides', c_u64 * 3), ('k1', N.c_u32),
        ('a2', N.c_void_p), ('a2_strides', c_u64 * 3), ('k2', N.c_u32),
        ('d1', N.c_u32), ('d2', N.c_u32), ('d3', N.c_u32), ('b1', N.c_u32), ('b2', N.c_u32), ('b3', N.c_u32),
        ('taps', N.c_u32),
        ('b', N.c_void_p), ('b_strides', c_u64 * 3), ('n', N.c_u32), ('n_rows_b', N.c_u32), ('bx2', N.c_u32), ('bx3', N.c_u32),
        ('b_batched', N.c_u32),
        ('bn', N.c_u32), ('alpha', N.c_f32), ('bias_n', N.c_void_p), ('residual', N.c_void_p),
        ('out', N.c_void_p), ('out_f32', N.c_u32), ('so1', c_ll), ('so2', c_ll), ('so3', c_ll),
        ('qstats', N.c_void_p), ('stats_hw', N.c_u32), ('algo', N.c_u32),
        ('tap_offsets', N.c_void_p), ('a_stride', N.c_u32), ('relu', N.c_u32),
    ]


ALGO_NARROW = 3


def _launch(a):
    N.check(N.lib().ssdnerf_gemm_f16(ctypes.byref(a), N.stream_ptr()))


def _pad_rows(w, mult=64):
    n = w.shape[-2]
    pad = (-n) % mult
    if pad:
        w = torch.cat([w, w.new_zeros(*w.shape[:-2], pad, w.shape[-1])], dim=-2)
    return w


def pack_linear_weight(w, narrow=False):
    w = w.detach().reshape(w.shape[0], -1).half()
    assert w.shape[1] % (8 if narrow else 64) == 0, 'K must be a multiple of 64 (narrow: of 8)'
    return _pad_rows(w).contiguous()


def pack_conv_weight(w, cin_pad=None, narrow=False):
    cout, cin = w.shape[0], w.shape[1]
    m = 8 if narrow else 64
    cin_pad = cin_pad or ((cin + m - 1) // m * m)
    wp = w.detach().permute(2, 3, 0, 1).reshape(9, cout, cin).half()
    if cin_pad != cin:
        wp = torch.cat([wp, wp.new_zeros(9, cout, cin_pad - cin)], dim=-1)
    return _pad_rows(wp).contiguous()


def linear_f16(a, w, bias=None, residual=None, out=None, out_f32=False, alpha=1.0, bn=0, n=None, qstats=None, stats_hw=0, narrow=False):
    N.require_cuda(a, w)
    M, K = a.shape
    n = n if n is not None else w.shape[0]
    if out is None:
        out = torch.empty(M, n, dtype=torch.float32 if out_f32 else torch.float16, device=a.device)
    g = GemmArgs()
    g.a1, g.k1 = a.data_ptr(), K
    rs = a.stride(0) * 2
    g.a1_strides = (c_u64 * 3)(rs, rs * M, rs * M)
    g.d1, g.d2, g.d3, g.b1, g.b2, g.b3 = M, 1, 1, 128, 1, 1
    g.taps = 1
    g.b, g.n, g.n_rows_b, g.bx2, g.bx3 = w.data_ptr(), n, w.shape[0], 1, 1
    ws = w.stride(0) * 2
    g.b_strides = (c_u64 * 3)(ws, ws * w.shape[0], ws * w.shape[0])
    g.bn, g.alpha = bn, alpha
    g.bias_n = bias.data_ptr() if bias is not None else None
    g.residual = residual.data_ptr() if residual is not None else None
    g.out, g.out_f32 = out.data_ptr(), int(out.dtype == torch.float32)
    g.so1, g.so2, g.so3 = out.stride(0), 0, 0
    if qstats is not None:
        g.qstats, g.stats_hw = qstats.data_ptr(), stats_hw
    if narrow:
        g.algo = ALGO_NARROW
    _launch(g)
    return out


def _conv_boxes(H, W, narrow=False):
    if narrow:
        return _conv_boxes_narrow(H, W)
    bw = min(W, 128)
    bh = min(H, 128 // bw)
    nb = 128 // (bw * bh)
    return bw, bh, nb


def _pow2_floor(v):
    return 1 << (max(int(v), 1).bit_length() - 1)


def _conv_boxes_narrow(H, W):
    bw = min(128, W & -W)
    bh = min(128 // bw, _pow2_floor(H))
    if 128 // (bw * bh) > 2:
        bw = min(128, 1 << (W - 1).bit_length())
        bh = min(128 // bw, 1 << (H - 1).bit_length())
    return bw, bh, 128 // (bw * bh)


def conv3x3_f16(x, wp, cout, bias=None, x2=None, residual=None, out=None, out_f32=False, taps=9, bn=0, qstats=None, algo=0, narrow=False,
                relu=False):
    N.require_cuda(x, wp)
    B, H, W, C1 = x.shape
    C2 = x2.shape[-1] if x2 is not None else 0
    assert x.is_contiguous() and (x2 is None or x2.is_contiguous())
    km = 8 if narrow else 64
    assert wp.shape[-1] == C1 + C2 and C1 % km == 0 and C2 % km == 0, (wp.shape, C1, C2)
    if narrow:
        algo = ALGO_NARROW
    if out is None:
        out = torch.empty(B, H, W, cout, dtype=torch.float32 if out_f32 else torch.float16, device=x.device)
    bw, bh, nb = _conv_boxes(H, W, narrow)
    g = GemmArgs()
    g.a1, g.k1 = x.data_ptr(), C1
    g.a1_strides = (c_u64 * 3)(C1 * 2, W * C1 * 2, H * W * C1 * 2)
    if x2 is not None:
        g.a2, g.k2 = x2.data_ptr(), C2
        g.a2_strides = (c_u64 * 3)(C2 * 2, W * C2 * 2, H * W * C2 * 2)
    g.d1, g.d2, g.d3, g.b1, g.b2, g.b3 = W, H, B, bw, bh, nb
    g.taps = taps
    ktot = C1 + C2
    rows = wp.shape[-2]
    g.b, g.n, g.n_rows_b, g.bx2, g.bx3 = wp.data_ptr(), cout, rows, taps, 1
    g.b_strides = (c_u64 * 3)(ktot * 2, rows * ktot * 2, taps * rows * ktot * 2)
    g.bn, g.alpha, g.algo = bn, 1.0, algo
    g.bias_n = bias.data_ptr() if bias is not None else None
    g.residual = residual.data_ptr() if residual is not None else None
    g.out, g.out_f32 = out.data_ptr(), int(out.dtype == torch.float32)
    co = out.shape[-1]
    g.so1, g.so2, g.so3 = co, W * co, H * W * co
    if qstats is not None:
        g.qstats, g.stats_hw = qstats.data_ptr(), 0
    g.relu = int(relu)
    _launch(g)
    return out


def conv3x3_s2_f16(x, wp, cout, bias=None, out=None, qstats=None, narrow=False):
    N.require_cuda(x, wp)
    B, H, W, C = x.shape
    assert x.is_contiguous() and H % 2 == 0 and W % 2 == 0 and wp.shape[-1] == C and C % (8 if narrow else 64) == 0
    Ho, Wo = H // 2, W // 2
    if out is None:
        out = torch.empty(B, Ho, Wo, cout, dtype=torch.float16, device=x.device)
    bw, bh, nb = _conv_boxes(Ho, Wo, narrow)
    g = GemmArgs()
    g.a1, g.k1 = x.data_ptr(), C
    g.a1_strides = (c_u64 * 3)(C * 2, W * C * 2, H * W * C * 2)
    g.d1, g.d2, g.d3, g.b1, g.b2, g.b3 = Wo, Ho, B, bw, bh, nb
    g.taps, g.a_stride = 9, 2
    rows = wp.shape[-2]
    g.b, g.n, g.n_rows_b, g.bx2, g.bx3 = wp.data_ptr(), cout, rows, 9, 1
    g.b_strides = (c_u64 * 3)(C * 2, rows * C * 2, 9 * rows * C * 2)
    g.bn, g.alpha, g.algo = 0, 1.0, ALGO_NARROW if narrow else 1
    g.bias_n = bias.data_ptr() if bias is not None else None
    g.out, g.out_f32 = out.data_ptr(), int(out.dtype == torch.float32)
    g.so1, g.so2, g.so3 = cout, Wo * cout, Ho * Wo * cout
    if qstats is not None:
        g.qstats, g.stats_hw = qstats.data_ptr(), 0
    _launch(g)
    return out


_UP_ROWS = {0: ((-1, (0,)), (0, (1, 2))), 1: ((0, (0, 1)), (1, (2,)))}


def pack_upconv_weight(w, narrow=False):
    w = w.detach().float()
    phases = []
    for py in (0, 1):
        for px in (0, 1):
            taps = []
            for _, kys in _UP_ROWS[py]:
                for _, kxs in _UP_ROWS[px]:
                    taps.append(sum(w[:, :, ky, kx] for ky in kys for kx in kxs))
            phases.append(torch.stack(taps))
    wp = torch.stack(phases).half()
    assert wp.shape[-1] % (8 if narrow else 64) == 0
    return _pad_rows(wp).contiguous()


def upconv3x3_f16(x, wps, cout, bias=None, out=None, qstats=None, narrow=False):
    N.require_cuda(x, wps)
    B, H, W, C = x.shape
    assert x.is_contiguous() and wps.shape[-1] == C
    if out is None:
        out = torch.empty(B, 2 * H, 2 * W, cout, dtype=torch.float16, device=x.device)
    bw, bh, nb = _conv_boxes(H, W, narrow)
    rows = wps.shape[-2]
    esz = out.element_size()
    for py in (0, 1):
        for px in (0, 1):
            offs = (ctypes.c_int8 * 8)(*[v for oy, _ in _UP_ROWS[py] for ox, _ in _UP_ROWS[px] for v in (ox, oy)])
            g = GemmArgs()
            g.a1, g.k1 = x.data_ptr(), C
            g.a1_strides = (c_u64 * 3)(C * 2, W * C * 2, H * W * C * 2)
            g.d1, g.d2, g.d3, g.b1, g.b2, g.b3 = W, H, B, bw, bh, nb
            g.taps, g.a_stride = 4, 1
            g.tap_offsets = ctypes.cast(offs, ctypes.c_void_p)
            ph = py * 2 + px
            g.b = wps.data_ptr() + ph * 4 * rows * C * 2
            g.n, g.n_rows_b, g.bx2, g.bx3 = cout, rows, 4, 1
            g.b_strides = (c_u64 * 3)(C * 2, rows * C * 2, 4 * rows * C * 2)
            g.bn, g.alpha, g.algo = 0, 1.0, ALGO_NARROW if narrow else 1
            g.bias_n = bias.data_ptr() if bias is not None else None
            g.out = out.data_ptr() + (py * 2 * W + px) * cout * esz
            g.out_f32 = int(out.dtype == torch.float32)
            g.so1, g.so2, g.so3 = 2 * cout, 2 * (2 * W) * cout, 4 * H * W * cout
            if qstats is not None:
                g.qstats, g.stats_hw = qstats.data_ptr(), 0
            _launch(g)
    return out


def attn_scores(qkv, heads, scale, out=None, narrow=False):
    B, T, c3 = qkv.shape
    c = c3 // 3
    ch = c // heads
    assert ch % (8 if narrow else 64) == 0
    if out is None:
        out = torch.empty(B, heads, T, T, dtype=torch.float32, device=qkv.device)
    g = GemmArgs()
    g.a1, g.k1 = qkv.data_ptr(), ch
    g.a1_strides = (c_u64 * 3)(c3 * 2, 3 * ch * 2, T * c3 * 2)
    g.d1, g.d2, g.d3, g.b1, g.b2, g.b3 = T, heads, B, 128, 1, 1
    g.taps = 1
    g.b = qkv.data_ptr() + ch * 2
    g.n, g.n_rows_b, g.bx2, g.bx3, g.b_batched = T, T, heads, B, 1
    g.b_strides = (c_u64 * 3)(c3 * 2, 3 * ch * 2, T * c3 * 2)
    g.bn, g.alpha = 0, scale
    g.out, g.out_f32 = out.data_ptr(), 1
    g.so1, g.so2, g.so3 = T, T * T, heads * T * T
    if narrow:
        g.algo = ALGO_NARROW
    _launch(g)
    return out


def attn_pv(P, vt, out=None, narrow=False):
    B, heads, T, _ = P.shape
    ch = vt.shape[2]
    c = heads * ch
    assert T % (8 if narrow else 64) == 0
    if out is None:
        out = torch.empty(B, T, c, dtype=torch.float16, device=P.device)
    g = GemmArgs()
    g.a1, g.k1 = P.data_ptr(), T
    g.a1_strides = (c_u64 * 3)(T * 2, T * T * 2, heads * T * T * 2)
    g.d1, g.d2, g.d3, g.b1, g.b2, g.b3 = T, heads, B, 128, 1, 1
    g.taps = 1
    g.b, g.n, g.n_rows_b, g.bx2, g.bx3, g.b_batched = vt.data_ptr(), ch, ch, heads, B, 1
    g.b_strides = (c_u64 * 3)(T * 2, ch * T * 2, heads * ch * T * 2)
    g.bn, g.alpha = 0, 1.0
    g.out, g.out_f32 = out.data_ptr(), 0
    g.so1, g.so2, g.so3 = c, ch, T * c
    if narrow:
        g.algo = ALGO_NARROW
    _launch(g)
    return out


def flash_attn(qkv, heads, scale, out=None):
    N.require_cuda(qkv)
    B, T, c3 = qkv.shape
    c = c3 // 3
    ch = c // heads
    assert qkv.is_contiguous() and qkv.dtype == torch.float16
    if out is None:
        out = torch.empty(B, T, c, dtype=torch.float16, device=qkv.device)
    N.check(N.lib().ssdnerf_flash_attn(N.ptr(qkv), N.c_u32(B), N.c_u32(T), N.c_u32(heads), N.c_u32(ch), N.c_f32(scale), N.ptr(out),
                                       N.stream_ptr()))
    return out


def pack_conv_weight_dgrad(w, cout_pad=None, narrow=False):
    return pack_conv_weight(w.detach().transpose(0, 1).flip(2, 3), cin_pad=cout_pad, narrow=narrow)


def pack_linear_weight_dgrad(w, narrow=False):
    w = w.detach().reshape(w.shape[0], -1)
    return pack_linear_weight(w.t(), narrow=narrow)


class GnBwdArgs(ctypes.Structure):
    _fields_ = [
        ('x1', N.c_void_p), ('C1', N.c_u32), ('x2', N.c_void_p), ('C2', N.c_u32), ('B', N.c_u32), ('HW', N.c_u32), ('groups', N.c_u32),
        ('stats', N.c_void_p), ('stats2', N.c_void_p), ('quad_stats', N.c_int), ('gamma', N.c_void_p), ('beta', N.c_void_p),
        ('scale_shift', N.c_void_p), ('ss_batch_stride', c_ll), ('eps', N.c_f32), ('do_silu', N.c_int),
        ('dy', N.c_void_p), ('add', N.c_void_p), ('group_sums', N.c_void_p), ('dx1', N.c_void_p), ('dx2', N.c_void_p),
        ('channel_sums', N.c_void_p),
    ]


def gn_bwd(x1, x2, stats, gamma, beta, dy, dx1, dx2=None, add=None, scale_shift_ptr=None, ss_batch_stride=0, silu=True, gsum=None, eps=1e-5,
           csum=None, groups=32):
    N.require_cuda(x1, dy, dx1)
    B, H, W, C1 = x1.shape
    a = GnBwdArgs()
    a.x1, a.C1 = x1.data_ptr(), C1
    if x2 is not None:
        a.x2, a.C2 = x2.data_ptr(), x2.shape[-1]
    a.B, a.HW, a.groups = B, H * W, groups
    quad, s1, s2 = stats
    a.stats, a.quad_stats = s1.data_ptr(), int(quad)
    a.stats2 = s2.data_ptr() if s2 is not None else None
    a.gamma, a.beta = gamma.data_ptr(), beta.data_ptr()
    if scale_shift_ptr is not None:
        a.scale_shift, a.ss_batch_stride = scale_shift_ptr, ss_batch_stride
    a.eps, a.do_silu = eps, int(silu)
    a.dy = dy.data_ptr()
    a.add = add.data_ptr() if add is not None else None
    if gsum is None:
        gsum = torch.empty(B * groups * 2, dtype=torch.float32, device=x1.device)
    a.group_sums = gsum.data_ptr()
    a.dx1 = dx1.data_ptr()
    a.dx2 = dx2.data_ptr() if dx2 is not None else None
    a.channel_sums = csum.data_ptr() if csum is not None else None
    N.check(N.lib().ssdnerf_gn_bwd(ctypes.byref(a), N.stream_ptr()))
    return dx1, dx2


class WgradArgs(ctypes.Structure):
    _fields_ = [
        ('gy', N.c_void_p), ('gy_stride', N.c_u32), ('gy_c0', N.c_u32),
        ('x', N.c_void_p), ('x_stride', N.c_u32), ('x_c0', N.c_u32),
        ('dw', N.c_void_p), ('dw_stride', N.c_u32), ('dw_c0', N.c_u32),
        ('batch', N.c_u32), ('out_h', N.c_u32), ('out_w', N.c_u32), ('in_h', N.c_u32), ('in_w', N.c_u32),
        ('cout', N.c_u32), ('cin', N.c_u32), ('taps', N.c_u32), ('stride', N.c_u32), ('up', N.c_int), ('ksplit', N.c_u32),
    ]


def conv_wgrad(gy, x, dw, cout, cin, taps=1, stride=1, up=False, gy_c0=0, x_c0=0, dw_c0=0, ksplit=0):
    N.require_cuda(gy, x, dw)
    assert gy.dtype == torch.float16 and x.dtype == torch.float16 and dw.dtype == torch.float32 and dw.is_contiguous()
    B, Ho, Wo, Cg = gy.shape
    _, Hi, Wi, Cx = x.shape
    a = WgradArgs()
    a.gy, a.gy_stride, a.gy_c0 = gy.data_ptr(), Cg, gy_c0
    a.x, a.x_stride, a.x_c0 = x.data_ptr(), Cx, x_c0
    a.dw, a.dw_stride, a.dw_c0 = dw.data_ptr(), dw.shape[-1], dw_c0
    a.batch, a.out_h, a.out_w, a.in_h, a.in_w = B, Ho, Wo, Hi, Wi
    a.cout, a.cin, a.taps, a.stride, a.up, a.ksplit = cout, cin, taps, stride, int(up), ksplit
    N.check(N.lib().ssdnerf_conv_wgrad_f16(ctypes.byref(a), N.stream_ptr()))
    return dw


def colsum(src, channels, out, c0=0):
    N.require_cuda(src, out)
    stride = src.shape[-1]
    N.check(N.lib().ssdnerf_colsum_f16(N.ptr(src), c_u64(src.numel() // stride), N.c_u32(stride), N.c_u32(c0), N.c_u32(channels),
                                       N.ptr(out), N.stream_ptr()))
    return out


def transpose_f16(src_ptr, dst, rows, cols, row_stride, stride1, n1, stride2, n2):
    N.check(N.lib().ssdnerf_transpose_f16(N.c_void_p(src_ptr), N.ptr(dst), N.c_u32(rows), N.c_u32(cols), c_ll(row_stride), c_ll(stride1),
                                          N.c_u32(n1), c_ll(stride2), N.c_u32(n2), N.stream_ptr()))
    return dst


def _bgemm(a_ptr, a_strides, k, b_ptr, b_strides, n, T, heads, B, out_ptr, out_strides, out_f32, alpha, narrow=False):
    g = GemmArgs()
    g.a1, g.k1 = a_ptr, k
    g.a1_strides = (c_u64 * 3)(*a_strides)
    g.d1, g.d2, g.d3, g.b1, g.b2, g.b3 = T, heads, B, 128, 1, 1
    g.taps = 1
    g.b, g.n, g.n_rows_b, g.bx2, g.bx3, g.b_batched = b_ptr, n, n, heads, B, 1
    g.b_strides = (c_u64 * 3)(*b_strides)
    g.bn, g.alpha = 0, alpha
    g.out, g.out_f32 = out_ptr, int(out_f32)
    g.so1, g.so2, g.so3 = out_strides
    if narrow:
        g.algo = ALGO_NARROW
    _launch(g)


def attn_backward(qkv, d_o, heads, scale, ws, narrow=False):
    B, T, c3 = qkv.shape
    c = c3 // 3
    ch = c // heads
    L, s = N.lib(), N.stream_ptr
    S = attn_scores(qkv, heads, scale, out=ws('S', (B, heads, T, T), torch.float32), narrow=narrow)
    P = ws('P', (B, heads, T, T), torch.float16)
    N.check(L.ssdnerf_softmax_rows(N.ptr(S), N.c_u32(B * heads * T), N.c_u32(T), N.ptr(P), s()))
    qp, dop = qkv.data_ptr(), d_o.data_ptr()
    TT = T * T
    _bgemm(dop, (c * 2, ch * 2, T * c * 2), ch, qp + 2 * ch * 2, (c3 * 2, 3 * ch * 2, T * c3 * 2), T, T, heads, B,
           S.data_ptr(), (T, TT, heads * TT), True, 1.0, narrow)
    dS = ws('dS', (B, heads, T, T), torch.float16)
    N.check(L.ssdnerf_softmax_bwd_rows(N.ptr(P), N.ptr(S), N.c_u32(B * heads * T), N.c_u32(T), N.ptr(dS), s()))
    Pt = transpose_f16(P.data_ptr(), ws('Pt', (B, heads, T, T), torch.float16), T, T, T, TT, heads, heads * TT, B)
    dSt = transpose_f16(dS.data_ptr(), ws('dSt', (B, heads, T, T), torch.float16), T, T, T, TT, heads, heads * TT, B)
    qt = transpose_f16(qp, ws('qt', (B, heads, ch, T), torch.float16), T, ch, c3, 3 * ch, heads, T * c3, B)
    kt = transpose_f16(qp + ch * 2, ws('kt', (B, heads, ch, T), torch.float16), T, ch, c3, 3 * ch, heads, T * c3, B)
    dot = transpose_f16(dop, ws('dot', (B, heads, ch, T), torch.float16), T, ch, c, ch, heads, T * c, B)
    dqkv = ws('dqkv', (B, T, c3), torch.float16)
    a_tt = (T * 2, TT * 2, heads * TT * 2)
    b_ct = (T * 2, ch * T * 2, heads * ch * T * 2)
    o_str = (c3, 3 * ch, T * c3)
    dp = dqkv.data_ptr()
    _bgemm(dS.data_ptr(), a_tt, T, kt.data_ptr(), b_ct, ch, T, heads, B, dp, o_str, False, scale, narrow)
    _bgemm(dSt.data_ptr(), a_tt, T, qt.data_ptr(), b_ct, ch, T, heads, B, dp + ch * 2, o_str, False, scale, narrow)
    _bgemm(Pt.data_ptr(), a_tt, T, dot.data_ptr(), b_ct, ch, T, heads, B, dp + 2 * ch * 2, o_str, False, 1.0, narrow)
    return dqkv


def dropout_f16(x, seed, p):
    if p <= 0:
        return x
    N.require_cuda(x)
    assert x.dtype == torch.float16 and x.is_contiguous()
    N.check(N.lib().ssdnerf_dropout_f16(N.ptr(x), ctypes.c_ulonglong(x.numel()), ctypes.c_ulonglong(seed & (2 ** 64 - 1)), N.c_f32(p),
                                        N.stream_ptr()))
    return x
```

Baseline: 97.56 million.

## Add split-K mode to the tensor-core GEMM for small UNet layers

Result: no change. 97.59 million (median of 6 runs) (+0.0%).

```diff
diff --git a/include/ssdnerf_b200.h b/include/ssdnerf_b200.h
--- a/include/ssdnerf_b200.h
+++ b/include/ssdnerf_b200.h
@@ -157,6 +157,9 @@
     uint32_t relu;
 } ssdnerf_gemm_args;
 SSDNERF_API int ssdnerf_gemm_f16(const ssdnerf_gemm_args* args, void* stream);
+SSDNERF_API int ssdnerf_gemm_f16_splitk(const ssdnerf_gemm_args* args, void* ws, size_t ws_bytes, void* stream);
+SSDNERF_API size_t ssdnerf_gemm_splitk_bytes(void);
+SSDNERF_API int ssdnerf_gemm_plan(const ssdnerf_gemm_args* args, const void* ws, size_t ws_bytes, int* out);
 
 SSDNERF_API int ssdnerf_nchw_to_nhwc_f16(const float* x, uint32_t B, uint32_t C, uint32_t H, uint32_t W, uint32_t Cpad, void* out, void* stream);
 SSDNERF_API int ssdnerf_gn_stats(const void* x1, uint32_t C1, const void* x2, uint32_t C2, uint32_t B, uint32_t HW, uint32_t groups,
diff --git a/ssdnerf_b200/_lib.py b/ssdnerf_b200/_lib.py
--- a/ssdnerf_b200/_lib.py
+++ b/ssdnerf_b200/_lib.py
@@ -62,7 +62,7 @@
         L = ctypes.CDLL(_PATH)
         L.ssdnerf_last_error.restype = ctypes.c_char_p
         for name in ('ssdnerf_decoder_blob_floats', 'ssdnerf_planes_bytes', 'ssdnerf_render_workspace_bytes',
-                     'ssdnerf_density_workspace_bytes', 'ssdnerf_unet_workspace_bytes'):
+                     'ssdnerf_density_workspace_bytes', 'ssdnerf_unet_workspace_bytes', 'ssdnerf_gemm_splitk_bytes'):
             if hasattr(L, name):
                 getattr(L, name).restype = c_size_t
         L.ssdnerf_mc_workspace_bytes.argtypes = [c_u32, c_u32, c_u32]
diff --git a/ssdnerf_b200/csrc/gemm_tc.cu b/ssdnerf_b200/csrc/gemm_tc.cu
--- a/ssdnerf_b200/csrc/gemm_tc.cu
+++ b/ssdnerf_b200/csrc/gemm_tc.cu
@@ -34,6 +34,9 @@
     float* qstats;
     uint32_t stats_hw;
     uint32_t k1, k2;
+    uint32_t splits;
+    float* part;
+    uint32_t* tile_cnt;
 };
 
 template <int BN>
@@ -45,11 +48,12 @@
                                     kMaxBiasN * 4 ;
 };
 
-template <int BN, bool KT, bool RELU = false>
+template <int BN, bool KT, bool RELU = false, bool SPLIT = false>
 __global__ void __launch_bounds__(kGemmThreads, 1)
 k_gemm_tc(const __grid_constant__ CUtensorMap mapA1, const __grid_constant__ CUtensorMap mapA2,
           const __grid_constant__ CUtensorMap mapB, const GemmParams p) {
     using Cfg = GemmCfg<BN>;
+    static_assert(!SPLIT || (!KT && !RELU && BN <= 128), "split K is built for the default family's 64 / 128-column tiles");
     extern __shared__ uint8_t smem_raw[];
     uint8_t* smem = reinterpret_cast<uint8_t*>(((uintptr_t)smem_raw + 1023) & ~(uintptr_t)1023);
     uint8_t* sA = smem;
@@ -62,9 +66,11 @@
     const int warp = threadIdx.x >> 5, lane = threadIdx.x & 31, wg = warp >> 2;
     const uint32_t tiles_m = p.T1 * p.T2 * p.T3;
     const uint32_t total_tiles = tiles_m * p.tiles_n;
-    const uint32_t iters = p.taps * (p.kc1 + p.kc2);
-    const uint32_t tile0 = blockIdx.x;
-    const uint32_t tile_step = gridDim.x;
+    const uint32_t kcc = p.kc1 + p.kc2;
+    const uint32_t iters = p.taps * kcc;
+    const uint32_t splits = SPLIT ? p.splits : 1u;
+    const uint32_t total_units = total_tiles * splits;
+    uint32_t* red_flag = reinterpret_cast<uint32_t*>(empty + Cfg::kStages);
 
     if (threadIdx.x == 0) {
         prefetch_tmap(&mapA1); prefetch_tmap(&mapA2); prefetch_tmap(&mapB);
@@ -81,21 +87,28 @@
         setmaxnreg_dec<40>();
         if (threadIdx.x == 0) {
             uint32_t stage = 0, phase = 0;
-            for (uint32_t tile = tile0; tile < total_tiles; tile += tile_step) {
+            for (uint32_t u = blockIdx.x; u < total_units; u += gridDim.x) {
+                const uint32_t tile = u / splits, split = u % splits;
                 const uint32_t m_tile = tile % tiles_m, n_tile = tile / tiles_m;
                 const uint32_t t1 = m_tile % p.T1, t2 = (m_tile / p.T1) % p.T2, t3 = m_tile / (p.T1 * p.T2);
-                for (uint32_t tap = 0; tap < p.taps; ++tap) {
-                    const int ox = p.tap_ox[tap], oy = p.tap_oy[tap];
-                    for (uint32_t j = 0; j < p.kc1 + p.kc2; ++j) {
-                        mbar_wait(&empty[stage], phase ^ 1);
-                        const bool first = j < p.kc1;
-                        const int ak = (int)((first ? j : j - p.kc1) * kBK), a1 = (int)(t1 * p.b1 * p.a_stride) + ox, a2 = (int)(t2 * p.b2 * p.a_stride) + oy, a3 = (int)(t3 * p.b3);
-                        mbar_expect_tx(&full[stage], (uint32_t)Cfg::kStageBytes);
-                        tma_load_4d(sA + stage * kABytes, first ? &mapA1 : &mapA2, &full[stage], ak, a1, a2, a3);
-                        const int bk = KT ? (first ? ak : (int)p.k1 + ak) : (int)(j * kBK);
-                        tma_load_4d(sB + stage * Cfg::kBBytes, &mapB, &full[stage], bk, (int)(n_tile * BN),
-                                    p.b_batched ? (int)t2 : (int)tap, p.b_batched ? (int)t3 : 0);
-                        if (++stage == Cfg::kStages) { stage = 0; phase ^= 1; }
+                auto issue = [&](uint32_t tap, uint32_t j, int ox, int oy) {
+                    mbar_wait(&empty[stage], phase ^ 1);
+                    const bool first = j < p.kc1;
+                    const int ak = (int)((first ? j : j - p.kc1) * kBK), a1 = (int)(t1 * p.b1 * p.a_stride) + ox, a2 = (int)(t2 * p.b2 * p.a_stride) + oy, a3 = (int)(t3 * p.b3);
+                    mbar_expect_tx(&full[stage], (uint32_t)Cfg::kStageBytes);
+                    tma_load_4d(sA + stage * kABytes, first ? &mapA1 : &mapA2, &full[stage], ak, a1, a2, a3);
+                    const int bk = KT ? (first ? ak : (int)p.k1 + ak) : (int)(j * kBK);
+                    tma_load_4d(sB + stage * Cfg::kBBytes, &mapB, &full[stage], bk, (int)(n_tile * BN),
+                                p.b_batched ? (int)t2 : (int)tap, p.b_batched ? (int)t3 : 0);
+                    if (++stage == Cfg::kStages) { stage = 0; phase ^= 1; }
+                };
+                if constexpr (SPLIT) {
+                    const uint32_t it0 = split * iters / splits, it1 = (split + 1) * iters / splits;
+                    for (uint32_t it = it0; it < it1; ++it) issue(it / kcc, it % kcc, p.tap_ox[it / kcc], p.tap_oy[it / kcc]);
+                } else {
+                    for (uint32_t tap = 0; tap < p.taps; ++tap) {
+                        const int ox = p.tap_ox[tap], oy = p.tap_oy[tap];
+                        for (uint32_t j = 0; j < kcc; ++j) issue(tap, j, ox, oy);
                     }
                 }
             }
@@ -109,14 +122,16 @@
         uint32_t stage = 0, phase = 0;
         float acc[BN / 2];
         auto release = [&](uint32_t s) { if (lane == 0) mbar_arrive(&empty[s]); };
-        for (uint32_t tile = tile0; tile < total_tiles; tile += tile_step) {
+        for (uint32_t u = blockIdx.x; u < total_units; u += gridDim.x) {
+            const uint32_t tile = u / splits, split = u % splits;
             const uint32_t m_tile = tile % tiles_m, n_tile = tile / tiles_m;
             const uint32_t t1 = m_tile % p.T1, t2 = (m_tile / p.T1) % p.T2, t3 = m_tile / (p.T1 * p.T2);
+            const uint32_t it0 = split * iters / splits, it1 = (split + 1) * iters / splits;
 #pragma unroll
             for (int i = 0; i < BN / 2; ++i) acc[i] = 0.0f;
             uint32_t prev = 0;
             uint32_t jc = 0;
-            for (uint32_t it = 0; it < iters; ++it) {
+            for (uint32_t it = it0; it < it1; ++it) {
                 mbar_wait(&full[stage], phase);
                 const uint64_t a_desc = make_desc_sw128(smem_u32(sA + stage * kABytes + cw * 64 * 128));
                 const uint64_t b_desc = make_desc_sw128(smem_u32(sB + stage * Cfg::kBBytes));
@@ -143,13 +158,39 @@
                 wgmma_commit();
                 fence_regs(acc);
                 wgmma_wait<1>();
-                if (it > 0) release(prev);
+                if (it > it0) release(prev);
                 prev = stage;
                 if (++stage == Cfg::kStages) { stage = 0; phase ^= 1; }
             }
             wgmma_wait<0>();
             fence_regs(acc);
-            if (iters > 0) release(prev);
+            if (it1 > it0) release(prev);
+
+            if constexpr (SPLIT) {
+                const uint32_t et = threadIdx.x - 128;
+                float4* mine = reinterpret_cast<float4*>(p.part) + (size_t)u * (BN / 8) * 256 + et;
+#pragma unroll
+                for (int i = 0; i < BN / 8; ++i) __stcg(mine + i * 256, make_float4(acc[4 * i], acc[4 * i + 1], acc[4 * i + 2], acc[4 * i + 3]));
+                __threadfence();
+                asm volatile("bar.sync 1, 256;" ::: "memory");
+                if (et == 0) {
+                    const bool last = atomicAdd(p.tile_cnt + tile, 1u) == splits - 1;
+                    if (last) p.tile_cnt[tile] = 0;
+                    *red_flag = last;
+                }
+                asm volatile("bar.sync 1, 256;" ::: "memory");
+                if (!*red_flag) continue;
+                __threadfence();
+                const float4* parts = reinterpret_cast<const float4*>(p.part) + (size_t)tile * splits * (BN / 8) * 256 + et;
+                for (uint32_t s = 0; s < splits; ++s) {
+#pragma unroll
+                    for (int i = 0; i < BN / 8; ++i) {
+                        const float4 q = __ldcg(parts + ((size_t)s * (BN / 8) + i) * 256);
+                        if (s == 0) { acc[4 * i] = q.x; acc[4 * i + 1] = q.y; acc[4 * i + 2] = q.z; acc[4 * i + 3] = q.w; }
+                        else { acc[4 * i] += q.x; acc[4 * i + 1] += q.y; acc[4 * i + 2] += q.z; acc[4 * i + 3] += q.w; }
+                    }
+                }
+            }
 
             long long off[2]; bool rok[2];
 #pragma unroll
@@ -167,45 +208,61 @@
                 img0 = p.stats_hw ? (t1 * p.b1) / p.stats_hw : t3 * p.b3;
                 slot = ((p.stats_hw ? (t1 * p.b1 + j1) / p.stats_hw : t3 * p.b3 + j3) - img0) & 1u;
             }
-#pragma unroll
-            for (int i = 0; i < BN / 8; ++i) {
-                const uint32_t c0 = 8u * i + 2u * cq;
-                const uint32_t ncol = n_tile * BN + c0;
-                const bool okc0 = ncol < p.n_valid, okc1 = ncol + 1 < p.n_valid;
-                float su = 0.0f, sq = 0.0f;
-#pragma unroll
-                for (int h = 0; h < 2; ++h) {
-                    float v0 = acc[4 * i + 2 * h] * p.alpha, v1 = acc[4 * i + 2 * h + 1] * p.alpha;
-                    if (!rok[h] || !okc0) continue;
-                    if (p.bias_n) { v0 += sbias[ncol]; if (okc1) v1 += sbias[ncol + 1]; }
-                    const long long o = off[h] + c0;
-                    if (p.residual) {
-                        if (p.vec2 && okc1) {
-                            const float2 r = __half22float2(*reinterpret_cast<const __half2*>(p.residual + o));
-                            v0 += r.x; v1 += r.y;
+            constexpr int kResChunk = 8;
+#pragma unroll
+            for (int i0 = 0; i0 < BN / 8; i0 += kResChunk) {
+                __half2 rv[kResChunk][2];
+#pragma unroll
+                for (int ii = 0; ii < kResChunk; ++ii) {
+#pragma unroll
+                    for (int h = 0; h < 2; ++h) {
+                        rv[ii][h] = __half2half2(__float2half_rn(0.0f));
+                        if (i0 + ii >= BN / 8 || !p.residual) continue;
+                        const uint32_t c0 = 8u * (i0 + ii) + 2u * cq;
+                        const uint32_t ncol = n_tile * BN + c0;
+                        if (!rok[h] || ncol >= p.n_valid) continue;
+                        const __half* rp = p.residual + off[h] + c0;
+                        if (p.vec2 && ncol + 1 < p.n_valid) rv[ii][h] = *reinterpret_cast<const __half2*>(rp);
+                        else rv[ii][h] = __halves2half2(rp[0], ncol + 1 < p.n_valid ? rp[1] : __float2half_rn(0.0f));
+                    }
+                }
+#pragma unroll
+                for (int ii = 0; ii < kResChunk; ++ii) {
+                    const int i = i0 + ii;
+                    if (i >= BN / 8) break;
+                    const uint32_t c0 = 8u * i + 2u * cq;
+                    const uint32_t ncol = n_tile * BN + c0;
+                    const bool okc0 = ncol < p.n_valid, okc1 = ncol + 1 < p.n_valid;
+                    float su = 0.0f, sq = 0.0f;
+#pragma unroll
+                    for (int h = 0; h < 2; ++h) {
+                        float v0 = acc[4 * i + 2 * h] * p.alpha, v1 = acc[4 * i + 2 * h + 1] * p.alpha;
+                        if (!rok[h] || !okc0) continue;
+                        if (p.bias_n) { v0 += sbias[ncol]; if (okc1) v1 += sbias[ncol + 1]; }
+                        const long long o = off[h] + c0;
+                        if (p.residual) {
+                            const float2 r = __half22float2(rv[ii][h]);
+                            v0 += r.x; if (okc1) v1 += r.y;
+                        }
+                        if constexpr (RELU) { v0 = fmaxf(v0, 0.0f); v1 = fmaxf(v1, 0.0f); }
+                        if (p.out_f32) {
+                            float* op = reinterpret_cast<float*>(p.out) + o;
+                            if (p.vec2 && okc1) *reinterpret_cast<float2*>(op) = make_float2(v0, v1);
+                            else { op[0] = v0; if (okc1) op[1] = v1; }
                         } else {
-                            v0 += __half2float(p.residual[o]);
-                            if (okc1) v1 += __half2float(p.residual[o + 1]);
+                            __half* op = reinterpret_cast<__half*>(p.out) + o;
+                            if (p.vec2 && okc1) *reinterpret_cast<__half2*>(op) = __floats2half2_rn(v0, v1);
+                            else { op[0] = __float2half_rn(v0); if (okc1) op[1] = __float2half_rn(v1); }
                         }
+                        if (!okc1) v1 = 0.0f;
+                        su += v0 + v1; sq = fmaf(v0, v0, fmaf(v1, v1, sq));
                     }
-                    if constexpr (RELU) { v0 = fmaxf(v0, 0.0f); v1 = fmaxf(v1, 0.0f); }
-                    if (p.out_f32) {
-                        float* op = reinterpret_cast<float*>(p.out) + o;
-                        if (p.vec2 && okc1) *reinterpret_cast<float2*>(op) = make_float2(v0, v1);
-                        else { op[0] = v0; if (okc1) op[1] = v1; }
-                    } else {
-                        __half* op = reinterpret_cast<__half*>(p.out) + o;
-                        if (p.vec2 && okc1) *reinterpret_cast<__half2*>(op) = __floats2half2_rn(v0, v1);
-                        else { op[0] = __float2half_rn(v0); if (okc1) op[1] = __float2half_rn(v1); }
-                    }
-                    if (!okc1) v1 = 0.0f;
-                    su += v0 + v1; sq = fmaf(v0, v0, fmaf(v1, v1, sq));
-                }
-                if (p.qstats) {
-                    frag_quad_reduce(su, sq);
-                    if ((lane & ~2) == 0) {
-                        float* qa = qacc + (slot * (BN / 4) + 2 * i + (lane >> 1)) * 2;
-                        atomicAdd(qa, su); atomicAdd(qa + 1, sq);
+                    if (p.qstats) {
+                        frag_quad_reduce(su, sq);
+                        if ((lane & ~2) == 0) {
+                            float* qa = qacc + (slot * (BN / 4) + 2 * i + (lane >> 1)) * 2;
+                            atomicAdd(qa, su); atomicAdd(qa + 1, sq);
+                        }
                     }
                 }
             }
@@ -270,15 +327,15 @@
 }
 int conv_row2_launch(const ssdnerf_gemm_args* a, int sms, cudaStream_t stream);
 
-template <int BN, bool KT = false, bool RELU = false>
+template <int BN, bool KT = false, bool RELU = false, bool SPLIT = false>
 static int launch_gemm(const CUtensorMap& mA1, const CUtensorMap& mA2, const CUtensorMap& mB, const GemmParams& p, int sms,
                        cudaStream_t stream) {
     using Cfg = GemmCfg<BN>;
     static DeviceOnce attr;
     if (attr.first()) {
-        SSDNERF_CUDA_OK(cudaFuncSetAttribute(k_gemm_tc<BN, KT, RELU>, cudaFuncAttributeMaxDynamicSharedMemorySize, (int)Cfg::kSmem));
-    }
-    const uint32_t total = p.T1 * p.T2 * p.T3 * p.tiles_n;
+        SSDNERF_CUDA_OK(cudaFuncSetAttribute(k_gemm_tc<BN, KT, RELU, SPLIT>, cudaFuncAttributeMaxDynamicSharedMemorySize, (int)Cfg::kSmem));
+    }
+    const uint32_t total = p.T1 * p.T2 * p.T3 * p.tiles_n * p.splits;
     cudaLaunchConfig_t cfg{};
     cfg.gridDim = dim3(total < (uint32_t)sms ? total : (uint32_t)sms);
     cfg.blockDim = dim3(kGemmThreads);
@@ -288,7 +345,7 @@
     at[0].id = cudaLaunchAttributeProgrammaticStreamSerialization;
     at[0].val.programmaticStreamSerializationAllowed = pdl_enabled() ? 1 : 0;
     cfg.attrs = at; cfg.numAttrs = 1;
-    SSDNERF_CUDA_OK(cudaLaunchKernelEx(&cfg, k_gemm_tc<BN, KT, RELU>, mA1, mA2, mB, p));
+    SSDNERF_CUDA_OK(cudaLaunchKernelEx(&cfg, k_gemm_tc<BN, KT, RELU, SPLIT>, mA1, mA2, mB, p));
     SSDNERF_LAUNCH_OK();
     return 0;
 }
@@ -297,8 +354,15 @@
 
 using namespace ssdnerf;
 
-extern "C" int ssdnerf_gemm_f16(const ssdnerf_gemm_args* a, void* stream_) {
-    cudaStream_t stream = (cudaStream_t)stream_;
+namespace {
+constexpr uint32_t kMaxSplits = 8, kMinSplitIters = 18;
+constexpr size_t kSplitCounterBytes = 4096;
+
+size_t splitk_bytes(int sms) { return kSplitCounterBytes + (size_t)sms * kBM * 256 * sizeof(float); }
+
+struct GemmPlan { int kernel = 0, bn = 0, splits = 1, grid = 0; };
+
+int plan_gemm(const ssdnerf_gemm_args* a, const void* ws, size_t ws_bytes, int sms, GemmPlan& pl) {
     if (!a || !a->a1 || !a->b || !a->out) return set_error_msg(SSDNERF_ERR_ARG, "gemm: a1, b and out are required");
     const bool kt = a->algo == 3;
     if (kt) {
@@ -315,13 +379,12 @@
     const uint32_t a_stride = a->a_stride == 2 ? 2u : 1u;
     if (a_stride == 2 && (a->b1 * 2 > 256 || a->b2 * 2 > 256)) return set_error_msg(SSDNERF_ERR_ARG, "gemm: stride-2 boxes exceed the 256-element TMA limit");
     if (a->n == 0 || a->d1 == 0 || a->d2 == 0 || a->d3 == 0) return 0;
-    int dev = 0, sms = 0;
-    SSDNERF_CUDA_OK(cudaGetDevice(&dev));
-    SSDNERF_CUDA_OK(cudaDeviceGetAttribute(&sms, cudaDevAttrMultiProcessorCount, dev));
     if (a->algo != 1 && !kt && !a->relu && a->taps == 9 && !a->tap_offsets && a_stride == 1 && a->d1 == 128 && a->b1 == 128 && a->b2 == 1 && a->b3 == 1 && a->n == 128 && !a->out_f32 && !a->b_batched &&
         (a->d2 % 2) == 0 && a->alpha == 1.0f && (a->bn == 0 || a->bn == 128) && a->so1 == 128 && a->so2 == 128 * 128 &&
-        a->so3 == (long long)a->d2 * 128 * 128 && (!a->qstats || a->stats_hw == 0) && (a->n_rows_b == 0 || a->n_rows_b >= 128))
-        return ssdnerf::conv_row2_launch(a, sms, stream);
+        a->so3 == (long long)a->d2 * 128 * 128 && (!a->qstats || a->stats_hw == 0) && (a->n_rows_b == 0 || a->n_rows_b >= 128)) {
+        pl.kernel = 2; pl.bn = 128;
+        return 0;
+    }
     if (a->algo == 2) return set_error_msg(SSDNERF_ERR_ARG, "gemm: algo 2 (row-pair convolution) needs taps 9, 128-pixel rows, 128 output channels, fp16 output");
     int bn = (int)a->bn;
     if (kt) {
@@ -340,19 +403,84 @@
                 for (int c : cand) { const uint32_t w = div_up(a->n, (uint32_t)c) * (uint32_t)c; if (w < best) { best = w; bn = c; } }
             }
         }
-    } else if (!bn) {
-        const uint32_t tiles_m = div_up(a->d1, a->b1) * div_up(a->d2, a->b2) * div_up(a->d3, a->b3);
+    }
+    const uint32_t tiles_m = div_up(a->d1, a->b1) * div_up(a->d2, a->b2) * div_up(a->d3, a->b3);
+    const uint32_t iters = a->taps * (div_up(a->k1, 64u) + (a->a2 ? div_up(a->k2, 64u) : 0));
+    const bool can_split = !kt && !a->relu && ws && ws_bytes >= splitk_bytes(sms);
+    auto splits_for = [&](uint32_t tiles, int tile_n) {
+        if (!can_split || tile_n > 128 || 2 * tiles > (uint32_t)sms) return 1u;
+        uint32_t s = (uint32_t)sms / tiles;
+        s = s < kMaxSplits ? s : kMaxSplits;
+        s = s < iters / kMinSplitIters ? s : iters / kMinSplitIters;
+        return s > 1 ? s : 1u;
+    };
+    auto pick_bn = [&](bool split) {
         double best = 1e30;
+        int pick = 0;
         const int cand[3] = {256, 128, 64};
         const double eff[3] = {1.0, 0.80, 0.50};
         for (int i = 0; i < 3; ++i) {
             if (cand[i] > 64 && (uint32_t)cand[i] / 2 >= a->n) continue;
             const uint32_t tiles = tiles_m * div_up(a->n, (uint32_t)cand[i]);
-            const double t = (double)div_up(tiles, (uint32_t)sms) * cand[i] / eff[i];
-            if (t < best) { best = t; bn = cand[i]; }
+            const uint32_t s = split ? splits_for(tiles, cand[i]) : 1u;
+            double t = (double)div_up(tiles * s, (uint32_t)sms) * cand[i] / eff[i];
+            if (s > 1) t *= (double)(div_up(iters, s) + 4 * s) / iters;
+            if (t < best) { best = t; pick = cand[i]; }
         }
+        return pick;
+    };
+    if (!kt && !bn) {
+        bn = pick_bn(false);
+        if (can_split && 2 * tiles_m * div_up(a->n, (uint32_t)bn) <= (uint32_t)sms) bn = pick_bn(true);
     }
     if (!kt && bn != 64 && bn != 128 && bn != 256) return set_error_msg(SSDNERF_ERR_ARG, "gemm: bn must be 64, 128 or 256");
+    if (a->bias_n && a->n > (uint32_t)kMaxBiasN) return set_error_msg(SSDNERF_ERR_ARG, "gemm: bias vectors longer than 2048 are not supported");
+    if (a->qstats && (a->n % 4)) return set_error_msg(SSDNERF_ERR_ARG, "gemm: quad statistics need n % 4 == 0");
+    if (a->qstats && !a->stats_hw && a->b3 > 2) return set_error_msg(SSDNERF_ERR_ARG, "gemm: fused quad statistics cover at most 2 images per 128-row tile (b3 <= 2)");
+    if (a->qstats && a->stats_hw && (a->stats_hw % 64)) return set_error_msg(SSDNERF_ERR_ARG, "gemm: stats_hw must be a multiple of 64");
+    pl.kernel = 1; pl.bn = bn;
+    const uint32_t tiles = tiles_m * div_up(a->n, (uint32_t)bn);
+    pl.splits = (int)splits_for(tiles, bn);
+    pl.grid = (int)(tiles * pl.splits < (uint32_t)sms ? tiles * pl.splits : (uint32_t)sms);
+    return 0;
+}
+
+int device_sms(int* sms) {
+    int dev = 0;
+    SSDNERF_CUDA_OK(cudaGetDevice(&dev));
+    SSDNERF_CUDA_OK(cudaDeviceGetAttribute(sms, cudaDevAttrMultiProcessorCount, dev));
+    return 0;
+}
+}
+
+extern "C" size_t ssdnerf_gemm_splitk_bytes(void) {
+    int sms = 0;
+    if (device_sms(&sms)) return 0;
+    return splitk_bytes(sms);
+}
+
+extern "C" int ssdnerf_gemm_plan(const ssdnerf_gemm_args* a, const void* ws, size_t ws_bytes, int* out) {
+    int sms = 0;
+    if (int e = device_sms(&sms)) return e;
+    GemmPlan pl;
+    if (int e = plan_gemm(a, ws, ws_bytes, sms, pl)) return e;
+    out[0] = pl.kernel; out[1] = pl.bn; out[2] = pl.splits; out[3] = pl.grid;
+    return 0;
+}
+
+extern "C" int ssdnerf_gemm_f16(const ssdnerf_gemm_args* a, void* stream) { return ssdnerf_gemm_f16_splitk(a, nullptr, 0, stream); }
+
+extern "C" int ssdnerf_gemm_f16_splitk(const ssdnerf_gemm_args* a, void* ws, size_t ws_bytes, void* stream_) {
+    cudaStream_t stream = (cudaStream_t)stream_;
+    int sms = 0;
+    if (int e = device_sms(&sms)) return e;
+    GemmPlan pl;
+    if (int e = plan_gemm(a, ws, ws_bytes, sms, pl)) return e;
+    if (pl.kernel == 0) return 0;
+    if (pl.kernel == 2) return ssdnerf::conv_row2_launch(a, sms, stream);
+    const bool kt = a->algo == 3;
+    const int bn = pl.bn;
+    const uint32_t a_stride = a->a_stride == 2 ? 2u : 1u;
 
     GemmParams p{};
     p.b1 = a->b1; p.b2 = a->b2; p.b3 = a->b3; p.d1 = a->d1; p.d2 = a->d2; p.d3 = a->d3;
@@ -369,12 +497,13 @@
     p.alpha = a->alpha; p.bias_n = a->bias_n; p.residual = (const __half*)a->residual; p.out = a->out; p.out_f32 = a->out_f32;
     p.so1 = a->so1; p.so2 = a->so2; p.so3 = a->so3;
     p.qstats = a->qstats; p.stats_hw = a->stats_hw;
+    p.splits = (uint32_t)pl.splits;
+    if (pl.splits > 1) {
+        p.tile_cnt = reinterpret_cast<uint32_t*>(ws);
+        p.part = reinterpret_cast<float*>(reinterpret_cast<uint8_t*>(ws) + kSplitCounterBytes);
+    }
     const uintptr_t pair_align = a->out_f32 ? 8u : 4u;
     p.vec2 = ((a->so1 | a->so2 | a->so3) & 1) == 0 && ((uintptr_t)a->out % pair_align) == 0 && ((uintptr_t)a->residual & 3u) == 0;
-    if (a->bias_n && a->n > (uint32_t)kMaxBiasN) return set_error_msg(SSDNERF_ERR_ARG, "gemm: bias vectors longer than 2048 are not supported");
-    if (a->qstats && (a->n % 4)) return set_error_msg(SSDNERF_ERR_ARG, "gemm: quad statistics need n % 4 == 0");
-    if (a->qstats && !a->stats_hw && a->b3 > 2) return set_error_msg(SSDNERF_ERR_ARG, "gemm: fused quad statistics cover at most 2 images per 128-row tile (b3 <= 2)");
-    if (a->qstats && a->stats_hw && (a->stats_hw % 64)) return set_error_msg(SSDNERF_ERR_ARG, "gemm: stats_hw must be a multiple of 64");
     const uint64_t ktot = (uint64_t)a->k1 + (a->a2 ? a->k2 : 0);
 
     CUtensorMap mA1, mA2, mB;
@@ -404,6 +533,10 @@
             default: return launch_gemm<16, true>(mA1, mA2, mB, p, sms, stream);
         }
     }
+    if (pl.splits > 1) {
+        if (bn == 128) return launch_gemm<128, false, false, true>(mA1, mA2, mB, p, sms, stream);
+        return launch_gemm<64, false, false, true>(mA1, mA2, mB, p, sms, stream);
+    }
     if (bn == 256) return launch_gemm<256>(mA1, mA2, mB, p, sms, stream);
     if (bn == 128) return launch_gemm<128>(mA1, mA2, mB, p, sms, stream);
     return launch_gemm<64>(mA1, mA2, mB, p, sms, stream);
diff --git a/ssdnerf_b200/unet.py b/ssdnerf_b200/unet.py
--- a/ssdnerf_b200/unet.py
+++ b/ssdnerf_b200/unet.py
@@ -307,6 +307,7 @@
         self.ss_cur = torch.zeros(batch, self.ss_total, dtype=torch.float32, device=dev)
         self.saving, self.tape, self.fwd_token, self._bwd_packed = False, [], 0, False
         self.drop_p, self._drop_seed = float(m.dropout), None
+        self.splitk_ws = U.splitk_workspace(dev)
         self.x_in = torch.zeros(batch, self.H, self.W, self.CPAD_IN, dtype=torch.float16, device=dev)
         self.v_out = torch.zeros(batch, self.H, self.W, self.out_conv['cout'], dtype=torch.float32, device=dev)
 
@@ -380,7 +381,7 @@
         nw = self.narrow
         if 'ws' in d:
             sc = U.conv3x3_f16(x, d['ws'].unsqueeze(0), cout, bias=d['wsb'], x2=sk, taps=1, out=self._buf(('sc', H, cout), (B, H, W, cout)),
-                               narrow=nw)
+                               narrow=nw, splitk_ws=self.splitk_ws)
         else:
             if sk is not None:
                 raise NotImplementedError('ResBlock with a skip concat but no shortcut convolution (cin + skip == cout) is not built')
@@ -390,13 +391,13 @@
         a = self._gn(x, qx, sk, qs, d['g1'], d['b1'], self._buf(('a', H, cin), (B, H, W, cin)), True)
         st1 = self._last_stats
         h1 = U.conv3x3_f16(a, d['w1'], cout, bias=d['c1b'], out=self._buf(('h1', tag) if self.saving else ('h1', H, cout), (B, H, W, cout)),
-                           qstats=qh1, narrow=nw)
+                           qstats=qh1, narrow=nw, splitk_ws=self.splitk_ws)
         a2 = self._gn(h1, qh1, None, None, d['g2'], d['b2'], self._buf(('a2', H, cout), (B, H, W, cout)), True, self.ss_offsets[d['idx']])
         st2 = self._last_stats
         if self.saving:
             self._dropout(a2, d['idx'])
         out = U.conv3x3_f16(a2, d['w2'], cout, bias=d['c2b'], residual=sc, out=self._buf(('res_out', tag), (B, H, W, cout)), qstats=qo,
-                            narrow=nw)
+                            narrow=nw, splitk_ws=self.splitk_ws)
         if self.saving:
             self.tape.append(dict(kind='res', d=d, x=x, sk=sk, st1=st1, h1=h1, st2=st2, out=out, tag=tag))
         return out, qo
@@ -410,11 +411,13 @@
         xn = self._gn(x, qx, None, None, d['g'], d['b'], self._buf(('xn', T, c), (B, H, W, c)), False)
         st = self._last_stats
         qkv = U.linear_f16(xn.view(B * T, c), d['wqkv'], bias=d['bqkv'], n=3 * c,
-                           out=self._buf(('qkv', tag) if self.saving else ('qkv', T, c), (B * T, 3 * c)), narrow=self.narrow)
+                           out=self._buf(('qkv', tag) if self.saving else ('qkv', T, c), (B * T, 3 * c)), narrow=self.narrow,
+                           splitk_ws=self.splitk_ws)
         o = self._attn_core(qkv, B, T, c, heads, ('o', T, c))
         qo = self._q(('attn_out', tag), c) if T % 64 == 0 else None
         out = U.linear_f16(o.view(B * T, c), d['wproj'], bias=d['bproj'], residual=x.view(B * T, c), n=c,
-                           out=self._buf(('attn_out', tag), (B * T, c)), qstats=qo, stats_hw=T, narrow=self.narrow).view(B, H, W, c)
+                           out=self._buf(('attn_out', tag), (B * T, c)), qstats=qo, stats_hw=T, narrow=self.narrow,
+                           splitk_ws=self.splitk_ws).view(B, H, W, c)
         if self.saving:
             self.tape.append(dict(kind='attn', d=d, x=x, st=st, qkv=qkv.view(B, T, 3 * c), out=out, tag=tag))
         return out, qo
@@ -436,7 +439,8 @@
         x, _ = x
         B, H, W, c = x.shape
         qo = self._q(('down_out', tag), c)
-        out = U.conv3x3_s2_f16(x, d['w'], c, bias=d['b'], out=self._buf(('down_out', tag), (B, H // 2, W // 2, c)), qstats=qo, narrow=self.narrow)
+        out = U.conv3x3_s2_f16(x, d['w'], c, bias=d['b'], out=self._buf(('down_out', tag), (B, H // 2, W // 2, c)), qstats=qo, narrow=self.narrow,
+                               splitk_ws=self.splitk_ws)
         if self.saving:
             self.tape.append(dict(kind='down', d=d, x=x, out=out, tag=tag))
         return out, qo
@@ -445,7 +449,8 @@
         x, _ = x
         B, H, W, c = x.shape
         qo = self._q(('up_out', tag), c)
-        out = U.upconv3x3_f16(x, d['w'], c, bias=d['b'], out=self._buf(('up_out', tag), (B, 2 * H, 2 * W, c)), qstats=qo, narrow=self.narrow)
+        out = U.upconv3x3_f16(x, d['w'], c, bias=d['b'], out=self._buf(('up_out', tag), (B, 2 * H, 2 * W, c)), qstats=qo, narrow=self.narrow,
+                              splitk_ws=self.splitk_ws)
         if self.saving:
             self.tape.append(dict(kind='up', d=d, x=x, out=out, tag=tag))
         return out, qo
diff --git a/ssdnerf_b200/unet_ops.py b/ssdnerf_b200/unet_ops.py
--- a/ssdnerf_b200/unet_ops.py
+++ b/ssdnerf_b200/unet_ops.py
@@ -26,8 +26,16 @@
 ALGO_NARROW = 3
 
 
-def _launch(a):
-    N.check(N.lib().ssdnerf_gemm_f16(ctypes.byref(a), N.stream_ptr()))
+def _launch(a, splitk_ws=None):
+    if splitk_ws is None:
+        N.check(N.lib().ssdnerf_gemm_f16(ctypes.byref(a), N.stream_ptr()))
+    else:
+        N.check(N.lib().ssdnerf_gemm_f16_splitk(ctypes.byref(a), N.c_void_p(splitk_ws.data_ptr()), N.c_size_t(splitk_ws.numel()),
+                                                N.stream_ptr()))
+
+
+def splitk_workspace(device):
+    return torch.zeros(int(N.lib().ssdnerf_gemm_splitk_bytes()), dtype=torch.uint8, device=device)
 
 
 def _pad_rows(w, mult=64):
@@ -54,7 +62,8 @@
     return _pad_rows(wp).contiguous()
 
 
-def linear_f16(a, w, bias=None, residual=None, out=None, out_f32=False, alpha=1.0, bn=0, n=None, qstats=None, stats_hw=0, narrow=False):
+def linear_f16(a, w, bias=None, residual=None, out=None, out_f32=False, alpha=1.0, bn=0, n=None, qstats=None, stats_hw=0, narrow=False,
+               splitk_ws=None):
     N.require_cuda(a, w)
     M, K = a.shape
     n = n if n is not None else w.shape[0]
@@ -78,7 +87,7 @@
         g.qstats, g.stats_hw = qstats.data_ptr(), stats_hw
     if narrow:
         g.algo = ALGO_NARROW
-    _launch(g)
+    _launch(g, splitk_ws)
     return out
 
 
@@ -105,7 +114,7 @@
 
 
 def conv3x3_f16(x, wp, cout, bias=None, x2=None, residual=None, out=None, out_f32=False, taps=9, bn=0, qstats=None, algo=0, narrow=False,
-                relu=False):
+                relu=False, splitk_ws=None):
     N.require_cuda(x, wp)
     B, H, W, C1 = x.shape
     C2 = x2.shape[-1] if x2 is not None else 0
@@ -138,11 +147,11 @@
     if qstats is not None:
         g.qstats, g.stats_hw = qstats.data_ptr(), 0
     g.relu = int(relu)
-    _launch(g)
-    return out
-
-
-def conv3x3_s2_f16(x, wp, cout, bias=None, out=None, qstats=None, narrow=False):
+    _launch(g, splitk_ws)
+    return out
+
+
+def conv3x3_s2_f16(x, wp, cout, bias=None, out=None, qstats=None, narrow=False, splitk_ws=None):
     N.require_cuda(x, wp)
     B, H, W, C = x.shape
     assert x.is_contiguous() and H % 2 == 0 and W % 2 == 0 and wp.shape[-1] == C and C % (8 if narrow else 64) == 0
@@ -164,7 +173,7 @@
     g.so1, g.so2, g.so3 = cout, Wo * cout, Ho * Wo * cout
     if qstats is not None:
         g.qstats, g.stats_hw = qstats.data_ptr(), 0
-    _launch(g)
+    _launch(g, splitk_ws)
     return out
 
 
@@ -186,7 +195,7 @@
     return _pad_rows(wp).contiguous()
 
 
-def upconv3x3_f16(x, wps, cout, bias=None, out=None, qstats=None, narrow=False):
+def upconv3x3_f16(x, wps, cout, bias=None, out=None, qstats=None, narrow=False, splitk_ws=None):
     N.require_cuda(x, wps)
     B, H, W, C = x.shape
     assert x.is_contiguous() and wps.shape[-1] == C
@@ -215,7 +224,7 @@
             g.so1, g.so2, g.so3 = 2 * cout, 2 * (2 * W) * cout, 4 * H * W * cout
             if qstats is not None:
                 g.qstats, g.stats_hw = qstats.data_ptr(), 0
-            _launch(g)
+            _launch(g, splitk_ws)
     return out
 
 
```
